# philipjesic/Distributed-Proof-Of-Work

Hardware: AMD Instinct MI355X
Metric: MD5 candidates/sec (GH/s), whole node (higher is better)
Workload: dtype u32; 1 GPU; sweep: nonce [1,2,3,4], 32 trailing zeros (unreachable), 2^36 candidates per GPU per step in the L=4 chunk segment (k >= 2^24); per-step RCCL MIN all-reduce; ntz=32, parallelism=prefix-partition x1 (workerBits=0)

## Files before the change

### distributed-proof-of-work_amd/csrc/dpow_api.cpp

```cpp
#include <hip/hip_runtime.h>
#include <stdio.h>
#include <stdlib.h>
#include <string.h>
#include <pthread.h>
#include <sched.h>
#include <sys/prctl.h>
#include <time.h>
#include <unistd.h>

#include <atomic>
#include <algorithm>
#include <chrono>
#include <mutex>
#include <string>
#include <thread>
#include <vector>

#include "../../include/dpow.h"
#include "../../include/dpow_worker.h"
#include "dpow_common.h"
#include "md5_host.h"
#include "md5_variants.h"
#include "node.h"
#include "plan.h"
#include "../../include/dpow_diag.h"


using namespace dpow;

namespace {

thread_local std::string g_last_error;

int set_error(int code, const std::string &msg) {
    g_last_error = msg;
    return code;
}

int hip_fail(hipError_t e, const char *what) {
    return set_error(DPOW_EHIP, std::string(what) + ": " + hipGetErrorString(e));
}

struct DeviceScope {
    int prev = -1;
    hipError_t e = hipSuccess;
    explicit DeviceScope(int dev) {
        if (hipGetDevice(&prev) != hipSuccess) prev = -1;
        if (prev != dev) e = hipSetDevice(dev);
        if (prev == dev) prev = -1;
    }
    ~DeviceScope() {
        if (prev >= 0) (void)hipSetDevice(prev);
    }
    DeviceScope(const DeviceScope &) = delete;
    DeviceScope &operator=(const DeviceScope &) = delete;
};

constexpr int DPOW_BOUNDED = 3;

#define DPOW_HIP(call)                                    \
    do {                                                  \
        hipError_t e_ = (call);                           \
        if (e_ != hipSuccess) return hip_fail(e_, #call); \
    } while (0)

constexpr uint64_t kBlocksPerCu = kMaxBlocksPerCu;
constexpr size_t kClaimRing = 64;
constexpr size_t kDepth = 3;
static_assert(kDepth < kClaimRing, "a claim slot is reused only after its launch completed");
constexpr size_t kRing = 8;
constexpr size_t kStaleWord = 8;
constexpr size_t kBoundWord = 16;
constexpr size_t kEarlyWord = 20;
constexpr size_t kCancelPage = 128;
static_assert(kEarlyWord * 4 + kCtrlRing * 8 <= kCancelPage, "the early-hit words fit the pinned page");
constexpr int64_t kSpinNs = 200000;
constexpr int64_t kSpinMaxNs = 4000000;
constexpr long kPollNs = 5000;
constexpr int64_t kNoDeadline = INT64_MAX;
constexpr int64_t kQueueLeadNs = 60000;
constexpr int64_t kEstFixedNs = 8000;

constexpr int kMaxDevices = 64;
std::atomic<int> g_active[kMaxDevices];
std::mutex g_ctx_mu;
std::vector<dpow_ctx *> g_ctxs;

struct ActiveSearch {
    int dev;
    explicit ActiveSearch(int d) : dev(d) { g_active[dev].fetch_add(1, std::memory_order_relaxed); }
    ~ActiveSearch() { g_active[dev].fetch_sub(1, std::memory_order_relaxed); }
};

struct LaunchSlot {
    uint64_t seq = 0;
    bool in_flight = false;
    uint64_t candidates = 0;
    uint64_t g_end = 0;
    hipStream_t stream = nullptr;
};

int64_t now_ns() {
    return std::chrono::duration_cast<std::chrono::nanoseconds>(std::chrono::steady_clock::now().time_since_epoch())
        .count();
}

struct SearchWait {
    int64_t t0 = now_ns();
    int64_t spin_ns = kSpinNs;
    long old_slack = -1;
    uint64_t node_seen = DPOW_NO_HIT;
    bool node_stop = false;
    const uint64_t *early = nullptr;
    uint64_t early_seen = DPOW_NO_HIT;
    uint64_t own_posted = DPOW_NO_HIT;
    uint64_t covered = 0;
    const uint8_t *nonce = nullptr;
    size_t nonce_len = 0;
    uint32_t ntz = 0;
    uint32_t rbits = 8, base_tb = 0;
    void lower_slack() {
        if (old_slack >= 0) return;
        const int r = prctl(PR_GET_TIMERSLACK, 0UL, 0UL, 0UL, 0UL);
        if (r <= 0) return;
        old_slack = r;
        (void)prctl(PR_SET_TIMERSLACK, 1000UL, 0UL, 0UL, 0UL);
    }
    ~SearchWait() {
        if (old_slack >= 0) (void)prctl(PR_SET_TIMERSLACK, (unsigned long)old_slack, 0UL, 0UL, 0UL);
    }
};

}

struct dpow_ctx {
    int device = 0;
    bool counted = false;
    hipStream_t stream = nullptr;
    Ctrl *d_ctrl = nullptr;
    Ctrl *d_ctrl_alloc = nullptr;
    uint32_t ctrl_idx = 0;
    unsigned long long *d_claims = nullptr;
    Snap *h_snap = nullptr;
    Snap *d_snap = nullptr;
    uint32_t *h_cancel = nullptr;
    uint32_t *d_cancel = nullptr;
    uint32_t cus = 0;
    uint64_t seq = 0;
    LaunchSlot slots[kRing];
    dpow_stats stats{};
    std::mutex bound_mu;
    bool searching = false;
    std::atomic<uint64_t> ext_bound{DPOW_NO_HIT};
    dpow_node_slot *node = nullptr;
    dpow_node_slot *d_node = nullptr;
    LaunchKnobs knobs;
    int64_t diag_t[8] = {0, 0, 0, 0, 0, 0, 0, 0};
    struct DiagLaunch {
        uint64_t seq = 0, candidates = 0, g_end = 0;
        int32_t kind = 0;
        int64_t queued = -1, seen = -1;
    };
    static constexpr size_t kDiagLaunches = 32;
    DiagLaunch diag_l[kDiagLaunches];
    size_t diag_nl = 0;
    int64_t diag_t0 = 0;
    uint64_t dev_key = 0;
    std::atomic<int64_t> last_use{0};
    bool solo = false;
};

namespace {

int retire_slot(dpow_ctx *c, LaunchSlot &s);

uint64_t *bound_word(dpow_ctx *c) { return reinterpret_cast<uint64_t *>(c->h_cancel + kBoundWord); }

int inject_bound_locked(dpow_ctx *c, uint64_t g) {
    if (g >= c->ext_bound.load(std::memory_order_relaxed)) return 0;
    c->ext_bound.store(g, std::memory_order_release);
    __atomic_store_n(bound_word(c), g, __ATOMIC_RELEASE);
    return 0;
}

int poll_node(dpow_ctx *c, SearchWait &sw) {
    dpow_node_slot *n = c->node;
    if (!n) return 0;
    const uint64_t nb = __atomic_load_n(&n->best, __ATOMIC_ACQUIRE);
    if (nb < sw.node_seen) {
        sw.node_seen = nb;
        if (nb != sw.own_posted) {
            std::lock_guard<std::mutex> g(c->bound_mu);
            uint64_t cur = c->ext_bound.load(std::memory_order_relaxed);
            if (nb < cur) c->ext_bound.store(nb, std::memory_order_release);
        }
    }
    if (!sw.node_stop && __atomic_load_n(&n->stop, __ATOMIC_ACQUIRE) != 0u) {
        sw.node_stop = true;
        __atomic_store_n(&c->h_cancel[kStaleWord], (uint32_t)c->seq, __ATOMIC_RELEASE);
    }
    return 0;
}

void poll_early(dpow_ctx *c, SearchWait &sw) {
    const uint64_t g = __atomic_load_n(sw.early, __ATOMIC_ACQUIRE);
    if (g >= sw.early_seen) return;
    sw.early_seen = g;
    if ((((uint32_t)g & 0xFFu) >> sw.rbits) != (sw.base_tb >> sw.rbits)) return;
    uint8_t sec[DPOW_MAX_SECRET];
    size_t len = 0;
    if (dpow_secret_from_index(g, sec, &len) != 0) return;
    if (!dpow_verify(sw.nonce, sw.nonce_len, sec, len, sw.ntz)) return;
    if (g < sw.own_posted) sw.own_posted = g;
    dpow_node_post(c->node, g);
    if (c->diag_t[7] < 0) c->diag_t[7] = now_ns() - sw.t0;
}

int wait_record(dpow_ctx *c, uint64_t seq, int64_t deadline, SearchWait &sw) {
    const uint32_t *p = &c->h_snap[seq % kRing].seq;
    const uint32_t want = (uint32_t)(seq + 1);
    for (uint64_t it = 1;; ++it) {
        if (__atomic_load_n(p, __ATOMIC_ACQUIRE) == want) return 1;
        const int64_t t = now_ns();
        if (t >= deadline) return 0;
        const bool spinning = t - sw.t0 < sw.spin_ns;
        if (spinning ? (it % 4096 == 0) : (it % 16 == 0)) {
            const hipError_t q = hipStreamQuery(c->slots[seq % kRing].stream);
            if (q == hipSuccess) {
                if (__atomic_load_n(p, __ATOMIC_ACQUIRE) == want) return 1;
                return set_error(DPOW_EHIP, "dpow_search: stream idle without the launch's completion record");
            }
            if (q != hipErrorNotReady) return hip_fail(q, "hipStreamQuery");
        }
        if (sw.early && (!spinning || it % 8 == 0)) poll_early(c, sw);
        if (!spinning || it % 64 == 0) {
            if (c->node) {
                const int rc = poll_node(c, sw);
                if (rc < 0) return rc;
            }
            if (c->ext_bound.load(std::memory_order_acquire) <= sw.covered) return 2;
        }
        if (spinning) {
            __builtin_ia32_pause();
        } else {
            sw.lower_slack();
            int64_t ns = kPollNs;
            if (deadline != kNoDeadline && deadline - t < ns) ns = deadline - t;
            const struct timespec ts = {0, (long)ns};
            nanosleep(&ts, nullptr);
        }
    }
}

int retire_slot(dpow_ctx *c, LaunchSlot &s) {
    if (!s.in_flight) return 0;
    const uint32_t *p = &c->h_snap[s.seq % kRing].seq;
    const uint32_t want = (uint32_t)(s.seq + 1);
    for (uint64_t it = 1; __atomic_load_n(p, __ATOMIC_ACQUIRE) != want; ++it) {
        if (it % 1024 == 0) {
            const hipError_t q = hipStreamQuery(s.stream);
            if (q == hipSuccess) {
                if (__atomic_load_n(p, __ATOMIC_ACQUIRE) == want) break;
                return set_error(DPOW_EHIP, "dpow_search: stream idle without a queued launch's completion record");
            }
            if (q != hipErrorNotReady) return hip_fail(q, "hipStreamQuery");
        }
        __builtin_ia32_pause();
    }
    s.in_flight = false;
    return 0;
}

int recent_contexts(int device) {
    const int64_t t = now_ns();
    int n = 0;
    std::lock_guard<std::mutex> g(g_ctx_mu);
    for (dpow_ctx *x : g_ctxs)
        if (x->device == device && t - x->last_use.load(std::memory_order_relaxed) < kRecentNs) ++n;
    return n;
}

int search_window(dpow_ctx *c, const uint8_t *nonce, size_t nonce_len, uint32_t ntz, uint32_t worker_byte,
                  uint32_t worker_bits, uint64_t k_begin, uint64_t k_end, uint64_t *best_global_idx,
                  uint8_t secret_out[DPOW_MAX_SECRET], size_t *secret_len) {
    WindowPlanner planner;
    int rc = planner.init(nonce, nonce_len, ntz, worker_byte, worker_bits, k_begin, k_end);
    if (rc < 0) return set_error(rc, "dpow_search: planning failed");
    const DeviceScope on_device(c->device);
    if (on_device.e != hipSuccess) return hip_fail(on_device.e, "hipSetDevice");
    if (c->device >= kMaxDevices) return set_error(DPOW_EINVAL, "dpow_search: device ordinal too large");
    const ActiveSearch active(c->device);
    SearchWait sw;
    {
        const double searches = (double)std::max(1, g_active[c->device].load(std::memory_order_relaxed));
        const double expect_ns =
            (double)expected_first_hit(ntz, remainder_bits(worker_bits)) / kEstRate * 1e9 * searches;
        sw.spin_ns = expect_ns > 2.0 * (double)kSpinMaxNs
                         ? kSpinNs
                         : (int64_t)std::min<double>(std::max<double>(2.0 * expect_ns, (double)kSpinNs),
                                                     (double)kSpinMaxNs);
    }

    {
        uint32_t *st = &c->h_cancel[kStaleWord];
        const uint32_t next = (uint32_t)(c->seq + 1);
        if ((int32_t)(next - __atomic_load_n(st, __ATOMIC_RELAXED)) > (1 << 30))
            __atomic_store_n(st, next - (1u << 30), __ATOMIC_RELAXED);
    }
    const uint64_t bound = *best_global_idx;
    const uint64_t node_best = c->node ? __atomic_load_n(&c->node->best, __ATOMIC_ACQUIRE) : DPOW_NO_HIT;
    sw.node_seen = node_best;
    const uint64_t seq0 = c->seq;
    sw.covered = k_begin << 8;
    for (int64_t &t : c->diag_t) t = -1;
    c->diag_nl = 0;
    c->diag_t0 = sw.t0;
    auto diag_queued = [c](size_t li, uint64_t seq, int32_t kind, uint64_t cands, uint64_t g_end) {
        if (li >= dpow_ctx::kDiagLaunches) return;
        c->diag_l[li] = {seq, cands, g_end, kind, now_ns(), -1};
        c->diag_nl = li + 1;
    };
    if (c->node) {
        uint64_t *ew = reinterpret_cast<uint64_t *>(c->h_cancel + kEarlyWord) + c->ctrl_idx;
        __atomic_store_n(ew, (uint64_t)DPOW_NO_HIT, __ATOMIC_RELEASE);
        sw.early = ew;
        sw.nonce = nonce;
        sw.nonce_len = nonce_len;
        sw.ntz = ntz;
        sw.rbits = remainder_bits(worker_bits);
        sw.base_tb = base_thread_byte(worker_byte, worker_bits);
    }
    size_t launched = 0, consumed = 0;
    int64_t busy_until = 0;
    PlannedLaunch pl;
    bool have = planner.next(pl);
    c->diag_t[4] = now_ns() - sw.t0;
    hipError_t e = hipSuccess;
    if (have && pl.k0) {
        LaunchSlot &k0slot = c->slots[seq0 % kRing];
        if ((rc = retire_slot(c, k0slot)) < 0) return rc;
        c->diag_t[5] = now_ns() - sw.t0;
        StartK0 k0{};
        k0.r = (uint32_t)(pl.L.i_end - pl.L.i_begin);
        k0.base_tb = pl.L.base_tb;
        k0.nblk = pl.info.nblk;
        k0.p = 4 * pl.info.w0 + pl.info.sh;
        k0.ntz = ntz;
        k0.seq = (uint32_t)(seq0 + 1);
        k0.snap = c->d_snap + seq0 % kRing;
        memcpy(k0.iv, pl.L.iv, sizeof k0.iv);
        memcpy(k0.T, pl.L.T, sizeof k0.T);
        e = search_k0(k0, c->stream);
        if (e != hipSuccess) return hip_fail(e, "search_k0");
        c->diag_t[0] = now_ns() - sw.t0;
        diag_queued(0, seq0, 0, k0.r, 1ull << 8);
        k0slot.in_flight = true;
        k0slot.seq = seq0;
        k0slot.candidates = k0.r;
        k0slot.g_end = 1ull << 8;
        k0slot.stream = c->stream;
        c->seq = seq0 + 1;
        launched = 1;
        have = planner.next(pl);
    }
    Ctrl *const ctrl = c->d_ctrl + (size_t)c->ctrl_idx * kCtrlStride;
    Ctrl *const ctrl_next = c->d_ctrl + (size_t)((c->ctrl_idx + 1) % kCtrlRing) * kCtrlStride;
    bool md5_queued = false;
    struct CtrlAdvance {
        dpow_ctx *c;
        const bool &queued;
        ~CtrlAdvance() {
            if (queued) c->ctrl_idx = (c->ctrl_idx + 1) % kCtrlRing;
        }
    } ctrl_advance{c, md5_queued};
    const uint64_t bound0 = node_best < bound ? node_best : bound;
    struct BoundWindow {
        dpow_ctx *c;
        BoundWindow(dpow_ctx *cc, uint64_t start) : c(cc) {
            std::lock_guard<std::mutex> g(c->bound_mu);
            c->ext_bound.store(start, std::memory_order_relaxed);
            __atomic_store_n(bound_word(c), (uint64_t)DPOW_NO_HIT, __ATOMIC_RELEASE);
            c->searching = true;
        }
        ~BoundWindow() {
            std::lock_guard<std::mutex> g(c->bound_mu);
            c->searching = false;
        }
    } bound_window(c, node_best);

    uint32_t done_target = 0;
    struct StaleOnReturn {
        dpow_ctx *c;
        const size_t &launched, &consumed;
        ~StaleOnReturn() {
            if (consumed < launched) __atomic_store_n(&c->h_cancel[kStaleWord], (uint32_t)c->seq, __ATOMIC_RELEASE);
        }
    } stale_on_return{c, launched, consumed};
    uint64_t best = bound;
    int status = DPOW_EXHAUSTED;
    auto consume = [&](size_t lj) -> int {
        const uint64_t seq = seq0 + lj;
        const int rc = wait_record(c, seq, kNoDeadline, sw);
        if (rc < 0) return rc;
        if (rc == 2) return DPOW_BOUNDED;
        LaunchSlot &slot = c->slots[seq % kRing];
        const Snap &sn = c->h_snap[seq % kRing];
        slot.in_flight = false;
        c->stats.launches++;
        c->stats.candidates += slot.candidates;
        if (sn.t_start != 0ull && sn.t_end >= sn.t_start)
            c->stats.kernel_ms += (double)(sn.t_end - sn.t_start) * kRealtimeNs * 1e-6;
        if (consumed == 0) c->diag_t[2] = now_ns() - sw.t0;
        if (lj < dpow_ctx::kDiagLaunches) c->diag_l[lj].seen = now_ns();
        consumed = lj + 1;
        if (c->node) {
            const int prc = poll_node(c, sw);
            if (prc < 0) return prc;
        }
        if (sn.best < bound) {
            const uint64_t eb = c->ext_bound.load(std::memory_order_acquire);
            if (sn.best >= eb) return eb <= slot.g_end ? DPOW_BOUNDED : DPOW_EXHAUSTED;
            best = sn.best;
            return DPOW_FOUND;
        }
        if (sn.stop != 0u || sw.node_stop || __atomic_load_n(c->h_cancel, __ATOMIC_ACQUIRE) != 0u)
            return DPOW_CANCELLED;
        sw.covered = slot.g_end;
        if (c->ext_bound.load(std::memory_order_acquire) <= sw.covered) return DPOW_BOUNDED;
        return DPOW_EXHAUSTED;
    };
    while (status == DPOW_EXHAUSTED && have) {
        if (sw.node_stop) {
            status = DPOW_CANCELLED;
            break;
        }
        const size_t li = launched;
        if (li - consumed >= kDepth) {
            const int r = consume(consumed);
            if (r < 0) return r;
            if (r != DPOW_EXHAUSTED) status = r;
            continue;
        }
        if (li > consumed && busy_until - now_ns() > kQueueLeadNs) {
            const size_t lj = consumed;
            const int w = wait_record(c, seq0 + lj, busy_until - kQueueLeadNs, sw);
            if (w < 0) return w;
            if (w == 2) {
                status = DPOW_BOUNDED;
                continue;
            }
            if (w == 1) {
                const int r = consume(lj);
                if (r < 0) return r;
                if (r != DPOW_EXHAUSTED) status = r;
                continue;
            }
        }
        {
            const uint64_t eb = c->ext_bound.load(std::memory_order_acquire);
            if ((pl.info.k_begin << 8) >= (eb < bound ? eb : bound)) break;
        }
        const uint64_t seq = seq0 + li;
        LaunchSlot &slot = c->slots[seq % kRing];
        if ((rc = retire_slot(c, slot)) < 0) return rc;
        if (!md5_queued) c->diag_t[6] = now_ns() - sw.t0;
        Launch &L = pl.L;
        uint64_t active = (uint64_t)std::max(1, g_active[c->device].load(std::memory_order_relaxed));
        if (active == 1 && !c->solo && now_ns() - sw.t0 < kYoungNs) {
            const int recent = recent_contexts(c->device);
            if (recent > 1) active = (uint64_t)recent;
        }
        const uint64_t share = grid_share(active, c->knobs);
        cap_shared_launch(planner, pl, active, c->knobs);
        uint64_t worker_blocks = 0;
        rc = size_search_launch(pl, ntz, c->cus, share, c->knobs, &worker_blocks, active);
        if (rc < 0) return set_error(rc, "dpow_search: launch grid leaves a claim counter without waves");
        done_target += (uint32_t)worker_blocks;
        L.claim = c->d_claims + (li % kClaimRing) * kClaimSlot;
        L.done_target = done_target;
        L.ctrl = ctrl;
        L.ctrl_next = ctrl_next;
        L.bound0 = bound0;
        L.cancel = c->d_cancel;
        L.stale = c->d_cancel + kStaleWord;
        L.ext_bound = reinterpret_cast<const unsigned long long *>(c->d_cancel + kBoundWord);
        L.snap = c->d_snap + seq % kRing;
        L.seq = (uint32_t)(seq + 1);
        L.node_best = c->d_node ? reinterpret_cast<const unsigned long long *>(&c->d_node->best) : nullptr;
        L.node_stop = c->d_node ? &c->d_node->stop : nullptr;
        L.early = c->d_node ? reinterpret_cast<unsigned long long *>(c->d_cancel + kEarlyWord) + c->ctrl_idx : nullptr;
        e = search_launch((int)pl.info.nblk, (int)pl.info.w0, (int)pl.info.sh, L, (uint32_t)(worker_blocks + 1),
                          c->stream);
        if (e != hipSuccess) return hip_fail(e, "search_launch");
        if (!md5_queued) c->diag_t[1] = now_ns() - sw.t0;
        diag_queued(li, seq, 1, L.i_end - L.i_begin, pl.info.k_end << 8);
        md5_queued = true;
        slot.seq = seq;
        slot.in_flight = true;
        slot.candidates = L.i_end - L.i_begin;
        slot.g_end = pl.info.k_end << 8;
        slot.stream = c->stream;
        c->seq = seq + 1;
        ++launched;
        const int64_t t = now_ns();
        busy_until = std::max(busy_until, t) + kEstFixedNs +
                     (int64_t)((double)slot.candidates * (double)active / kEstRate * 1e9);
        have = planner.next(pl);
    }
    while (status == DPOW_EXHAUSTED && consumed < launched) {
        const int r = consume(consumed);
        if (r < 0) return r;
        status = r;
    }
    if (status == DPOW_BOUNDED) status = DPOW_EXHAUSTED;
    c->diag_t[3] = now_ns() - sw.t0;

    if (status == DPOW_FOUND) {
        dpow_secret_from_index(best, secret_out, secret_len);
        if (!dpow_verify(nonce, nonce_len, secret_out, *secret_len, ntz)) {
            *secret_len = 0;
            return set_error(DPOW_EVERIFY, "dpow_search: kernel hit failed host MD5 verification");
        }
        *best_global_idx = best;
    }
    return status;
}

struct PageEntry {
    void *page;
    bool foreign;
    std::vector<dpow_ctx *> holders;
    char *dev[kMaxDevices] = {};
};
std::mutex g_page_mu;
std::vector<PageEntry> g_pages;

void page_drop_locked(size_t i) {
    if (!g_pages[i].foreign) (void)hipHostUnregister(g_pages[i].page);
    g_pages.erase(g_pages.begin() + (long)i);
}

hipError_t page_hold_locked(dpow_ctx *c, void *page, char **dev) {
    PageEntry *pe = nullptr;
    for (PageEntry &x : g_pages)
        if (x.page == page) {
            pe = &x;
            break;
        }
    if (!pe) {
        hipError_t e = hipHostRegister(page, 4096, hipHostRegisterMapped | hipHostRegisterPortable);
        bool foreign = false;
        if (e == hipErrorHostMemoryAlreadyRegistered) {
            (void)hipGetLastError();
            e = hipSuccess;
            foreign = true;
        }
        if (e != hipSuccess) return e;
        g_pages.push_back(PageEntry{page, foreign, {}, {}});
        pe = &g_pages.back();
    }
    if (!pe->dev[c->device]) {
        void *d = nullptr;
        const hipError_t e = hipHostGetDevicePointer(&d, page, 0);
        if (e != hipSuccess) {
            if (pe->holders.empty()) page_drop_locked((size_t)(pe - g_pages.data()));
            return e;
        }
        pe->dev[c->device] = static_cast<char *>(d);
    }
    if (std::find(pe->holders.begin(), pe->holders.end(), c) == pe->holders.end()) pe->holders.push_back(c);
    *dev = pe->dev[c->device];
    return hipSuccess;
}

void pages_release_ctx(dpow_ctx *c) {
    std::lock_guard<std::mutex> g(g_page_mu);
    for (size_t i = g_pages.size(); i-- > 0;) {
        auto &h = g_pages[i].holders;
        h.erase(std::remove(h.begin(), h.end(), c), h.end());
        if (h.empty()) page_drop_locked(i);
    }
}

hipError_t prepare_device(int device) {
    static std::mutex mu;
    static bool prepared[kMaxDevices] = {};
    std::lock_guard<std::mutex> g(mu);
    if (device < kMaxDevices && prepared[device]) return hipSuccess;
    const hipError_t e = search_prepare();
    if (e == hipSuccess && device < kMaxDevices) prepared[device] = true;
    return e;
}

}

extern "C" {

const char *dpow_last_error(void) { return g_last_error.c_str(); }
int dpow_abi_version(void) { return DPOW_ABI_VERSION; }

int dpow_device_count(void) {
    int n = 0;
    if (hipGetDeviceCount(&n) != hipSuccess) {
        (void)hipGetLastError();
        return 0;
    }
    return n;
}

int dpow_open(int device, dpow_ctx **out) {
    if (!out) return set_error(DPOW_EINVAL, "dpow_open: out is NULL");
    *out = nullptr;
    int n = 0;
    hipError_t e = hipGetDeviceCount(&n);
    if (e != hipSuccess || n == 0) return set_error(DPOW_EHIP, "dpow_open: no HIP device visible");
    if (device < 0 || device >= n) return set_error(DPOW_EINVAL, "dpow_open: bad device ordinal");
    const DeviceScope on_device(device);
    if (on_device.e != hipSuccess) return hip_fail(on_device.e, "hipSetDevice");
    dpow_ctx *c = new (std::nothrow) dpow_ctx();
    if (!c) return set_error(DPOW_ENOMEM, "dpow_open: out of memory");
    c->device = device;
    hipDeviceProp_t prop;
    if ((e = hipGetDeviceProperties(&prop, device)) != hipSuccess) {
        delete c;
        return hip_fail(e, "hipGetDeviceProperties");
    }
    c->cus = (uint32_t)prop.multiProcessorCount;
    {
        char bus[64] = {0};
        if (hipDeviceGetPCIBusId(bus, (int)sizeof bus - 1, device) != hipSuccess) {
            (void)hipGetLastError();
            snprintf(bus, sizeof bus, "ordinal-%d-pid-%d", device, (int)getpid());
        }
        uint64_t h = 1469598103934665603ull;
        for (const char *q = bus; *q; ++q) h = (h ^ (uint8_t)*q) * 1099511628211ull;
        c->dev_key = h | 1ull;
    }
    if (const char *pw = getenv("DPOW_DIAG_POLL_WB")) c->knobs.poll_wb = (uint32_t)std::max(0, atoi(pw));
    if (const char *pw = getenv("DPOW_DIAG_BPC")) c->knobs.bpc = (uint32_t)std::max(0, atoi(pw));
    if (const char *pw = getenv("DPOW_DIAG_CPW")) c->knobs.cpw = (uint32_t)std::max(0, atoi(pw));
    if (const char *pw = getenv("DPOW_DIAG_SHARE_LAUNCH_US")) c->knobs.share_launch_us = (uint32_t)std::max(0, atoi(pw));
    if (const char *pw = getenv("DPOW_DIAG_SHARE_MAX")) c->knobs.share_max = (uint32_t)std::max(0, atoi(pw));
    if (const char *pw = getenv("DPOW_DIAG_MIN_CHUNK")) {
        const uint32_t v = (uint32_t)std::max(0, atoi(pw));
        if (v && !(v & (v - 1))) c->knobs.min_chunk = v;
    }
    if ((e = hipStreamCreateWithFlags(&c->stream, hipStreamNonBlocking)) != hipSuccess ||
        (e = hipMalloc(&c->d_ctrl_alloc, 2 * kCtrlRing * kCtrlStride * sizeof(Ctrl))) != hipSuccess ||
        (e = hipMalloc(&c->d_claims, kClaimRing * kClaimSlot * sizeof(unsigned long long))) != hipSuccess ||
        (e = hipHostMalloc(&c->h_snap, kRing * sizeof(Snap), hipHostMallocCoherent | hipHostMallocMapped)) !=
            hipSuccess ||
        (e = hipHostGetDevicePointer(reinterpret_cast<void **>(&c->d_snap), c->h_snap, 0)) != hipSuccess ||
        (e = hipHostMalloc(&c->h_cancel, kCancelPage, hipHostMallocCoherent | hipHostMallocMapped)) != hipSuccess ||
        (e = hipHostGetDevicePointer(reinterpret_cast<void **>(&c->d_cancel), c->h_cancel, 0)) != hipSuccess) {
        dpow_close(c);
        return hip_fail(e, "dpow_open: allocation");
    }
    {
        const uintptr_t rb = kCtrlRing * kCtrlStride * sizeof(Ctrl);
        c->d_ctrl = reinterpret_cast<Ctrl *>((reinterpret_cast<uintptr_t>(c->d_ctrl_alloc) + rb - 1) & ~(rb - 1));
    }
    memset(c->h_snap, 0, kRing * sizeof(Snap));
    memset(c->h_cancel, 0, kCancelPage);
    *bound_word(c) = DPOW_NO_HIT;
    if ((e = context_init(c->d_ctrl, kCtrlRing * kCtrlStride, c->d_claims, (uint32_t)(kClaimRing * kClaimSlot),
                          c->stream)) != hipSuccess ||
        (e = hipStreamSynchronize(c->stream)) != hipSuccess) {
        dpow_close(c);
        return hip_fail(e, "dpow_open: control state");
    }
    if ((e = prepare_device(device)) != hipSuccess) {
        dpow_close(c);
        return hip_fail(e, "dpow_open: loading the search kernels");
    }
    c->last_use.store(now_ns(), std::memory_order_relaxed);
    {
        std::lock_guard<std::mutex> g(g_ctx_mu);
        g_ctxs.push_back(c);
        c->counted = true;
    }
    *out = c;
    return 0;
}

void dpow_close(dpow_ctx *c) {
    if (!c) return;
    if (c->counted) {
        std::lock_guard<std::mutex> g(g_ctx_mu);
        g_ctxs.erase(std::remove(g_ctxs.begin(), g_ctxs.end(), c), g_ctxs.end());
    }
    const DeviceScope on_device(c->device);
    if (c->stream) (void)hipStreamSynchronize(c->stream);
    c->node = c->d_node = nullptr;
    pages_release_ctx(c);
    if (c->d_ctrl_alloc) (void)hipFree(c->d_ctrl_alloc);
    if (c->d_claims) (void)hipFree(c->d_claims);
    if (c->h_snap) (void)hipHostFree(c->h_snap);
    if (c->h_cancel) (void)hipHostFree(c->h_cancel);
    if (c->stream) (void)hipStreamDestroy(c->stream);
    delete c;
}

volatile uint32_t *dpow_cancel_flag(dpow_ctx *c) { return c ? c->h_cancel : nullptr; }
void *dpow_stream(dpow_ctx *c) { return c ? (void *)c->stream : nullptr; }
int dpow_device(dpow_ctx *c) { return c ? c->device : -1; }

int dpow_geometry(dpow_ctx *c, uint32_t *cus, uint32_t *blocks_per_cu, uint32_t *threads_per_block) {
    if (!c) return set_error(DPOW_EINVAL, "dpow_geometry: ctx is NULL");
    if (cus) *cus = c->cus;
    if (blocks_per_cu) *blocks_per_cu = (uint32_t)kBlocksPerCu;
    if (threads_per_block) *threads_per_block = kBlockThreads;
    return 0;
}

int dpow_get_stats(dpow_ctx *c, dpow_stats *out) {
    if (!c || !out) return set_error(DPOW_EINVAL, "dpow_get_stats: NULL argument");
    *out = c->stats;
    return 0;
}

void dpow_reset_stats(dpow_ctx *c) {
    if (!c) return;
    c->stats = dpow_stats{};
}

int dpow_search_bound(dpow_ctx *c, uint64_t global_idx) {
    if (!c) return set_error(DPOW_EINVAL, "dpow_search_bound: ctx is NULL");
    std::lock_guard<std::mutex> g(c->bound_mu);
    if (!c->searching) return 0;
    return inject_bound_locked(c, global_idx);
}

int dpow_node_attach(dpow_ctx *c, dpow_node_slot *slot) {
    if (!c) return set_error(DPOW_EINVAL, "dpow_node_attach: ctx is NULL");
    if (!slot) {
        c->node = c->d_node = nullptr;
        return 0;
    }
    if (((uintptr_t)slot & 7u) != 0u) return set_error(DPOW_EINVAL, "dpow_node_attach: slot not 8-byte aligned");
    if (c->device >= kMaxDevices) return set_error(DPOW_EINVAL, "dpow_node_attach: device ordinal too large");
    const DeviceScope on_device(c->device);
    if (on_device.e != hipSuccess) return hip_fail(on_device.e, "hipSetDevice");
    const uintptr_t pg = 4096;
    const bool one_page = (((uintptr_t)slot & (pg - 1)) + sizeof(dpow_node_slot)) <= pg;
    char *dev = nullptr;
    {
        std::lock_guard<std::mutex> g(g_page_mu);
        for (uintptr_t a = (uintptr_t)slot & ~(pg - 1); a < (uintptr_t)slot + sizeof(dpow_node_slot); a += pg) {
            char *d = nullptr;
            const hipError_t e = page_hold_locked(c, (void *)a, &d);
            if (e != hipSuccess) return hip_fail(e, "dpow_node_attach: hipHostRegister");
            if (!dev) dev = d;
        }
    }
    void *d = dev + ((uintptr_t)slot & (pg - 1));
    if (!one_page) DPOW_HIP(hipHostGetDevicePointer(&d, slot, 0));
    c->node = slot;
    c->d_node = (dpow_node_slot *)d;
    return 0;
}

int dpow_node_release(void *mem, size_t len) {
    if (!mem || !len) return 0;
    const uintptr_t pg = 4096;
    const uintptr_t lo = (uintptr_t)mem & ~(pg - 1), hi = (uintptr_t)mem + len;
    std::lock_guard<std::mutex> g(g_page_mu);
    for (const PageEntry &pe : g_pages) {
        const uintptr_t p = (uintptr_t)pe.page;
        if (p < lo || p >= hi) continue;
        for (dpow_ctx *h : pe.holders)
            if (h->node && (uintptr_t)h->node < p + pg && (uintptr_t)h->node + sizeof(dpow_node_slot) > p)
                return set_error(DPOW_EINVAL, "dpow_node_release: a context is still attached to a slot in the range");
    }
    for (size_t i = g_pages.size(); i-- > 0;) {
        const uintptr_t p = (uintptr_t)g_pages[i].page;
        if (p < lo || p >= hi) continue;
        for (dpow_ctx *h : g_pages[i].holders) {
            const DeviceScope on_device(h->device);
            const hipError_t e = hipStreamSynchronize(h->stream);
            if (e != hipSuccess) return hip_fail(e, "dpow_node_release: hipStreamSynchronize");
        }
        page_drop_locked(i);
    }
    return 0;
}

void dpow_node_slot_reset(dpow_node_slot *slot) {
    if (!slot) return;
    __atomic_store_n(&slot->stop, 0u, __ATOMIC_RELAXED);
    __atomic_store_n(&slot->best, DPOW_NO_HIT, __ATOMIC_RELEASE);
}

void dpow_node_post(dpow_node_slot *slot, uint64_t global_idx) {
    if (!slot) return;
    uint64_t cur = __atomic_load_n(&slot->best, __ATOMIC_RELAXED);
    while (global_idx < cur &&
           !__atomic_compare_exchange_n(&slot->best, &cur, global_idx, true, __ATOMIC_ACQ_REL, __ATOMIC_RELAXED)) {
    }
}

int dpow_node_vote(dpow_node_vote_entry *votes, uint32_t rank, uint32_t world, uint64_t epoch, const int64_t in[3],
                   int64_t out[3], int64_t timeout_ns) {
    return dpow::node_vote(votes, rank, world, epoch, in, out, timeout_ns, nullptr);
}

}

int dpow::node_vote(dpow_node_vote_entry *votes, uint32_t rank, uint32_t world, uint64_t epoch, const int64_t in[3],
                    int64_t out[3], int64_t timeout_ns, const uint32_t *abort_flag) {
    if (!votes || !in || !out || world == 0 || rank >= world || epoch == 0)
        return set_error(DPOW_EINVAL, "dpow_node_vote: bad argument");
    dpow_node_vote_entry &mine = votes[2 * rank + (epoch & 1)];
    for (int i = 0; i < 3; ++i) __atomic_store_n(&mine.v[i], in[i], __ATOMIC_RELAXED);
    __atomic_store_n(&mine.epoch, epoch, __ATOMIC_RELEASE);
    int64_t acc[3] = {in[0], in[1], in[2]};
    const int64_t t0 = now_ns();
    constexpr int64_t kVoteSpinNs = 500000;
    long old_slack = -1;
    struct SlackRestore {
        long &old;
        ~SlackRestore() {
            if (old >= 0) (void)prctl(PR_SET_TIMERSLACK, (unsigned long)old, 0UL, 0UL, 0UL);
        }
    } slack_restore{old_slack};
    for (uint32_t r = 0; r < world; ++r) {
        if (r == rank) continue;
        const dpow_node_vote_entry &e = votes[2 * r + (epoch & 1)];
        for (uint64_t it = 0; __atomic_load_n(&e.epoch, __ATOMIC_ACQUIRE) != epoch; ++it) {
            if (abort_flag && it % 64 == 0 && __atomic_load_n(abort_flag, __ATOMIC_ACQUIRE) != 0u) return DPOW_CANCELLED;
            if (it % 64 != 0 || now_ns() - t0 < std::min(kVoteSpinNs, timeout_ns)) {
                __builtin_ia32_pause();
                continue;
            }
            if (now_ns() - t0 > timeout_ns)
                return set_error(DPOW_EPROTO, "dpow_node_vote: rank " + std::to_string(r) + " did not vote at epoch " +
                                                  std::to_string(epoch));
            if (old_slack < 0) {
                const int sl = prctl(PR_GET_TIMERSLACK, 0UL, 0UL, 0UL, 0UL);
                if (sl > 0) {
                    old_slack = sl;
                    (void)prctl(PR_SET_TIMERSLACK, 1000UL, 0UL, 0UL, 0UL);
                }
            }
            const struct timespec d = {0, 2000};
            nanosleep(&d, nullptr);
        }
        for (int i = 0; i < 3; ++i) {
            const int64_t v = __atomic_load_n(&e.v[i], __ATOMIC_RELAXED);
            if (v < acc[i]) acc[i] = v;
        }
    }
    for (int i = 0; i < 3; ++i) out[i] = acc[i];
    return 0;
}

extern "C" int dpow_node_mine(dpow_ctx *c, dpow_node_slot *slot, dpow_node_vote_entry *votes, uint32_t rank,
                              uint32_t world, uint64_t *epoch, int64_t vote_timeout_ns, const uint8_t *nonce,
                              size_t nonce_len, uint32_t ntz, uint64_t k_begin, uint64_t k_limit, uint64_t first_k,
                              uint64_t batch_k, uint64_t *best_global_idx, uint8_t secret_out[DPOW_MAX_SECRET],
                              size_t *secret_len, uint32_t *batches) {
    return dpow::node_mine(c, slot, votes, rank, world, epoch, vote_timeout_ns, nonce, nonce_len, ntz, k_begin, k_limit,
                           first_k, batch_k, best_global_idx, secret_out, secret_len, batches, false, 0);
}

int dpow::node_mine(dpow_ctx *c, dpow_node_slot *slot, dpow_node_vote_entry *votes, uint32_t rank, uint32_t world,
                    uint64_t *epoch, int64_t vote_timeout_ns, const uint8_t *nonce, size_t nonce_len, uint32_t ntz,
                    uint64_t k_begin, uint64_t k_limit, uint64_t first_k, uint64_t batch_k, uint64_t *best_global_idx,
                    uint8_t secret_out[DPOW_MAX_SECRET], size_t *secret_len, uint32_t *batches, bool abandon_on_cancel,
                    int role) {
    if (!c || !slot || !epoch || !best_global_idx || !secret_out || !secret_len || !batches)
        return set_error(DPOW_EINVAL, "dpow_node_mine: NULL argument");
    if (world == 0 || (world & (world - 1)) != 0 || world > 256 || rank >= world)
        return set_error(DPOW_EINVAL, "dpow_node_mine: world must be a power of two <= 256, rank < world");
    if (batch_k == 0 || k_limit > DPOW_K_LIMIT) return set_error(DPOW_EINVAL, "dpow_node_mine: bad window");
    const uint32_t wbits = (uint32_t)__builtin_ctz(world);
    *batches = 0;
    *secret_len = 0;
    int err = dpow_node_attach(c, slot);
    if (err < 0) dpow_node_stop(slot);
    uint64_t k = k_begin, window = first_k ? first_k : batch_k;
    uint8_t sec[DPOW_MAX_SECRET];
    size_t slen = 0;
    uint64_t own = DPOW_NO_HIT;
    int status = DPOW_EXHAUSTED;
    while (k < k_limit) {
        const uint64_t ke = k_limit - k > window ? k + window : k_limit;
        window = batch_k;
        int rc = DPOW_EXHAUSTED;
        if (err == 0) {
            uint64_t best = DPOW_NO_HIT;
            if (role == 2) rc = DPOW_EXHAUSTED;
            else rc = dpow_search(c, nonce, nonce_len, ntz, role == 1 ? 0 : rank, role == 1 ? 0 : wbits, k, ke, &best,
                                  sec, &slen);
            if (rc < 0) {
                err = rc;
                dpow_node_stop(slot);
            } else if (rc == DPOW_FOUND && best < own) {
                own = best;
                memcpy(secret_out, sec, slen);
                *secret_len = slen;
            }
        }
        const int64_t running =
            (err != 0 || rc == DPOW_CANCELLED || __atomic_load_n(c->h_cancel, __ATOMIC_ACQUIRE) != 0u) ? 0 : 1;
        const uint64_t posted = __atomic_load_n(&slot->best, __ATOMIC_ACQUIRE);
        const int64_t in[3] = {(int64_t)(own < posted ? own : posted), running, err != 0 ? 0 : 1};
        int64_t out[3] = {in[0], in[1], in[2]};
        if (abandon_on_cancel && err == 0 && __atomic_load_n(c->h_cancel, __ATOMIC_ACQUIRE) != 0u) {
            dpow_node_stop(slot);
            status = DPOW_CANCELLED;
            break;
        }
        if (votes) {
            const int vr = node_vote(votes, rank, world, ++*epoch, in, out, vote_timeout_ns,
                                     abandon_on_cancel ? c->h_cancel : nullptr);
            if (vr == DPOW_CANCELLED) {
                dpow_node_stop(slot);
                status = DPOW_CANCELLED;
                break;
            }
            if (vr < 0) {
                err = err ? err : vr;
                out[2] = 0;
            }
        }
        ++*batches;
        if (out[2] == 0) {
            status = err ? err : set_error(DPOW_EPROTO, "dpow_node_mine: another rank's search failed");
            break;
        }
        if ((uint64_t)out[0] != DPOW_NO_HIT) {
            *best_global_idx = (uint64_t)out[0];
            if ((uint64_t)out[0] != own) dpow_secret_from_index((uint64_t)out[0], secret_out, secret_len);
            status = DPOW_FOUND;
            break;
        }
        if (out[1] == 0) {
            status = DPOW_CANCELLED;
            break;
        }
        k = ke;
    }
    if (c->node == slot) c->node = c->d_node = nullptr;
    if (status != DPOW_FOUND) *secret_len = 0;
    return status;
}

int dpow::fail(int code, const char *msg) { return set_error(code, msg); }

uint64_t dpow::device_key(const dpow_ctx *c) { return c ? c->dev_key : 0; }

void dpow::set_solo(dpow_ctx *c, bool solo) {
    if (c) c->solo = solo;
}

extern "C" {

int dpow_diag_node_post_at(dpow_node_slot *slot, uint64_t global_idx, int64_t t_ns) {
    if (!slot) return set_error(DPOW_EINVAL, "dpow_diag_node_post_at: slot is NULL");
    struct Poster {
        std::mutex mu;
        std::vector<std::pair<int64_t, std::pair<dpow_node_slot *, uint64_t>>> q;
        std::atomic<int> pending{0};
        bool alive = false;
    };
    static Poster *const P = new Poster;
    std::lock_guard<std::mutex> g(P->mu);
    P->q.push_back({t_ns, {slot, global_idx}});
    P->pending.fetch_add(1, std::memory_order_release);
    if (!P->alive) {
        P->alive = true;
        std::thread([]() {
            auto mono = []() {
                struct timespec ts;
                clock_gettime(CLOCK_MONOTONIC, &ts);
                return (int64_t)ts.tv_sec * 1000000000 + ts.tv_nsec;
            };
            int64_t idle_since = mono();
            for (;;) {
                if (P->pending.load(std::memory_order_acquire) == 0) {
                    if (mono() - idle_since > 2000000000) {
                        std::lock_guard<std::mutex> g2(P->mu);
                        if (P->pending.load(std::memory_order_acquire) == 0) {
                            P->alive = false;
                            return;
                        }
                    }
                    __builtin_ia32_pause();
                    continue;
                }
                std::pair<int64_t, std::pair<dpow_node_slot *, uint64_t>> w;
                int rest = 0;
                {
                    std::lock_guard<std::mutex> g2(P->mu);
                    auto it = std::min_element(P->q.begin(), P->q.end(),
                                               [](const auto &x, const auto &y) { return x.first < y.first; });
                    w = *it;
                    P->q.erase(it);
                    rest = P->pending.fetch_sub(1, std::memory_order_acq_rel) - 1;
                }
                bool requeued = false;
                for (;;) {
                    const int64_t left = w.first - mono();
                    if (left <= 0) break;
                    if (P->pending.load(std::memory_order_acquire) > rest) {
                        std::lock_guard<std::mutex> g2(P->mu);
                        P->q.push_back(w);
                        P->pending.fetch_add(1, std::memory_order_release);
                        requeued = true;
                        break;
                    }
                    if (left > 100000) {
                        const struct timespec d = {0, (long)std::min<int64_t>(left - 50000, 50000)};
                        nanosleep(&d, nullptr);
                    } else {
                        __builtin_ia32_pause();
                    }
                }
                if (requeued) continue;
                dpow_node_post(w.second.first, w.second.second);
                idle_since = mono();
            }
        }).detach();
    }
    return 0;
}

int dpow_diag_vote_latency(uint32_t world, int reps, double *last_us, double *all_us) {
    if (world < 2 || world > 256 || reps < 1 || !last_us || !all_us)
        return set_error(DPOW_EINVAL, "dpow_diag_vote_latency: world in [2, 256], reps >= 1, outputs non-NULL");
    void *mem = aligned_alloc(64, (size_t)2 * world * sizeof(dpow_node_vote_entry));
    if (!mem) return set_error(DPOW_EINVAL, "dpow_diag_vote_latency: out of memory");
    memset(mem, 0, (size_t)2 * world * sizeof(dpow_node_vote_entry));
    auto *votes = static_cast<dpow_node_vote_entry *>(mem);
    cpu_set_t allowed;
    CPU_ZERO(&allowed);
    std::vector<int> cpus;
    if (sched_getaffinity(0, sizeof allowed, &allowed) == 0)
        for (int i = 0; i < CPU_SETSIZE; ++i) {
            if (!CPU_ISSET(i, &allowed)) continue;
            char path[96];
            snprintf(path, sizeof path, "/sys/devices/system/cpu/cpu%d/topology/thread_siblings_list", i);
            if (FILE *f = fopen(path, "r")) {
                int first = -1;
                const int n = fscanf(f, "%d", &first);
                fclose(f);
                if (n == 1 && first != i) continue;
            }
            cpus.push_back(i);
        }
    auto pin = [&](uint32_t r) {
        if (cpus.empty()) return;
        cpu_set_t one;
        CPU_ZERO(&one);
        CPU_SET(cpus[(size_t)r * cpus.size() / world], &one);
        (void)pthread_setaffinity_np(pthread_self(), sizeof one, &one);
    };
    std::atomic<int> go{0};
    std::vector<std::atomic<int64_t>> done_at(world);
    for (auto &d : done_at) d.store(0);
    std::atomic<int> failed{0};
    std::vector<std::thread> others;
    for (uint32_t r = 1; r < world; ++r)
        others.emplace_back([&, r]() {
            pin(r);
            for (int rep = 1; rep <= reps; ++rep) {
                while (go.load(std::memory_order_acquire) < rep) __builtin_ia32_pause();
                if (failed.load()) break;
                const int64_t in[3] = {(int64_t)(1000 + r), 1, 1};
                int64_t out[3];
                if (dpow_node_vote(votes, r, world, (uint64_t)rep, in, out, 1000000000) != 0) failed.store(1);
                done_at[r].store(now_ns(), std::memory_order_release);
                while (go.load(std::memory_order_acquire) == rep) __builtin_ia32_pause();
            }
        });
    cpu_set_t caller;
    const bool have_caller = pthread_getaffinity_np(pthread_self(), sizeof caller, &caller) == 0;
    pin(0);
    std::vector<double> last, all;
    int64_t t_prev_done = 0;
    for (int rep = 1; rep <= reps && !failed.load(); ++rep) {
        go.store(rep, std::memory_order_release);
        for (uint32_t r = 1; r < world; ++r)
            while (__atomic_load_n(&votes[2 * r + (rep & 1)].epoch, __ATOMIC_ACQUIRE) != (uint64_t)rep &&
                   !failed.load())
                __builtin_ia32_pause();
        for (const int64_t t_wait = now_ns(); now_ns() - t_wait < 2000;) __builtin_ia32_pause();
        const int64_t t0 = now_ns();
        const int64_t in[3] = {1000, 1, 1};
        int64_t out[3];
        if (dpow_node_vote(votes, 0, world, (uint64_t)rep, in, out, 1000000000) != 0 || out[0] != 1000) failed.store(1);
        const int64_t t1 = now_ns();
        int64_t t_all = t1;
        for (uint32_t r = 1; r < world && !failed.load(); ++r) {
            int64_t t;
            while ((t = done_at[r].load(std::memory_order_acquire)) <= t_prev_done && !failed.load())
                __builtin_ia32_pause();
            t_all = std::max(t_all, t);
        }
        t_prev_done = t_all;
        last.push_back((t1 - t0) / 1e3);
        all.push_back((t_all - t0) / 1e3);
    }
    go.store(reps + 1, std::memory_order_release);
    for (auto &t : others) t.join();
    if (have_caller) (void)pthread_setaffinity_np(pthread_self(), sizeof caller, &caller);
    free(mem);
    if (failed.load() || last.empty()) return set_error(DPOW_EPROTO, "dpow_diag_vote_latency: a vote failed");
    std::sort(last.begin(), last.end());
    std::sort(all.begin(), all.end());
    *last_us = last[last.size() / 2];
    *all_us = all[all.size() / 2];
    return 0;
}

void dpow_node_stop(dpow_node_slot *slot) {
    if (slot) __atomic_store_n(&slot->stop, 1u, __ATOMIC_RELEASE);
}

int dpow_secret_from_index(uint64_t g, uint8_t secret_out[DPOW_MAX_SECRET], size_t *secret_len) {
    if (!secret_out || !secret_len) return set_error(DPOW_EINVAL, "dpow_secret_from_index: NULL argument");
    if (g == DPOW_NO_HIT) return set_error(DPOW_EINVAL, "dpow_secret_from_index: no hit");
    size_t n = 0;
    secret_out[n++] = (uint8_t)(g & 0xFF);
    for (uint64_t k = g >> 8; k; k >>= 8) secret_out[n++] = (uint8_t)(k & 0xFF);
    *secret_len = n;
    return 0;
}

void dpow_md5(const uint8_t *msg, size_t len, uint8_t digest_out[16]) { md5_digest(msg, len, digest_out); }

uint32_t dpow_trailing_zero_nibbles(const uint8_t digest[16]) { return digest_trailing_zero_nibbles(digest); }

int dpow_verify(const uint8_t *nonce, size_t nonce_len, const uint8_t *secret, size_t secret_len, uint32_t ntz) {
    std::vector<uint8_t> msg(nonce_len + secret_len);
    if (nonce_len) memcpy(msg.data(), nonce, nonce_len);
    if (secret_len) memcpy(msg.data() + nonce_len, secret, secret_len);
    uint8_t d[16];
    md5_digest(msg.data(), msg.size(), d);
    return digest_trailing_zero_nibbles(d) >= ntz ? 1 : 0;
}

int dpow_plan_window(const uint8_t *nonce, size_t nonce_len, uint32_t ntz, uint32_t worker_byte,
                     uint32_t worker_bits, uint64_t k_begin, uint64_t k_end, dpow_plan_launch *out,
                     size_t max_launches) {
    std::vector<PlannedLaunch> plan;
    int n = plan_window(nonce, nonce_len, ntz, worker_byte, worker_bits, k_begin, k_end, plan);
    if (n < 0) return set_error(n, "dpow_plan_window: bad arguments");
    for (size_t i = 0; i < plan.size() && i < max_launches && out; ++i) out[i] = plan[i].info;
    return n;
}

int dpow_plan_candidate(const uint8_t *nonce, size_t nonce_len, uint32_t worker_byte, uint32_t worker_bits,
                        uint64_t local_idx, uint32_t iv_out[4], uint32_t words_out[32], uint32_t *nblk_out) {
    if (!iv_out || !words_out || !nblk_out) return set_error(DPOW_EINVAL, "dpow_plan_candidate: NULL argument");
    const uint64_t k = local_idx >> remainder_bits(worker_bits);
    const uint32_t clen = chunk_len_of(k);
    uint64_t k_first = clen == 0 ? k : 1ull << (8 * (clen - 1));
    if (const uint64_t w2 = word2_period((uint32_t)(nonce_len % 64) % 4))
        if (k_first < k / w2 * w2) k_first = k / w2 * w2;
    std::vector<PlannedLaunch> plan;
    int n = plan_window(nonce, nonce_len, 0, worker_byte, worker_bits, k_first, k + 1, plan);
    if (n != 1) return set_error(n < 0 ? n : DPOW_EINVAL, "dpow_plan_candidate: bad arguments");
    for (int w = 0; w < 4; ++w) iv_out[w] = plan[0].L.iv[w];
    memset(words_out, 0, 32 * sizeof(uint32_t));
    candidate_words(plan[0], local_idx, words_out);
    *nblk_out = plan[0].info.nblk;
    return 0;
}

int dpow_diag_launch_geometry(const uint8_t *nonce, size_t nonce_len, uint32_t ntz, uint32_t worker_byte,
                              uint32_t worker_bits, uint64_t k_begin, uint64_t k_end, uint32_t cus, uint32_t share,
                              dpow_diag_launch *out, size_t max_launches) {
    if (cus == 0 || share == 0) return set_error(DPOW_EINVAL, "dpow_diag_launch_geometry: cus and share must be > 0");
    WindowPlanner planner;
    const int rc = planner.init(nonce, nonce_len, ntz, worker_byte, worker_bits, k_begin, k_end);
    if (rc < 0) return set_error(rc, "dpow_diag_launch_geometry: bad arguments");
    PlannedLaunch pl;
    size_t n = 0;
    const LaunchKnobs policy{};
    while (planner.next(pl)) {
        if (pl.k0) continue;
        cap_shared_launch(planner, pl, share, policy);
        uint64_t wblocks = 0;
        const int r = size_search_launch(pl, ntz, cus, grid_share(share, policy), policy, &wblocks, share);
        if (r < 0) return set_error(r, "dpow_diag_launch_geometry: launch grid leaves a claim counter without waves");
        if (out && n < max_launches) {
            dpow_diag_launch &d = out[n];
            d.k_begin = pl.info.k_begin;
            d.k_end = pl.info.k_end;
            d.i_begin = pl.L.i_begin;
            d.i_end = pl.L.i_end;
            d.wb_begin = pl.L.wb_begin;
            d.n_wblocks = pl.L.n_wblocks;
            d.n_big = pl.L.n_big;
            d.n_chunks = pl.L.n_chunks;
            d.worker_blocks = wblocks;
            d.chunk = pl.L.chunk;
            d.chunk_tail = pl.L.chunk_tail;
            d.rbits = pl.L.rbits;
            d.wave_block = kWaveBlock;
            d.n_static = pl.L.n_static;
            d.poll_wb = pl.L.poll_wb;
        }
        ++n;
    }
    return (int)n;
}

int dpow_diag_node_alias(dpow_ctx *c, void **cached, void **lookup) {
    if (!c || !cached || !lookup) return set_error(DPOW_EINVAL, "dpow_diag_node_alias: NULL argument");
    if (!c->node) return set_error(DPOW_EINVAL, "dpow_diag_node_alias: no slot attached");
    const DeviceScope on_device(c->device);
    if (on_device.e != hipSuccess) return hip_fail(on_device.e, "hipSetDevice");
    *cached = c->d_node;
    DPOW_HIP(hipHostGetDevicePointer(lookup, c->node, 0));
    return 0;
}

int dpow_diag_search_times(dpow_ctx *c, int64_t out[8]) {
    if (!c || !out) return set_error(DPOW_EINVAL, "dpow_diag_search_times: NULL argument");
    for (int i = 0; i < 8; ++i) out[i] = c->diag_t[i];
    return 0;
}

int dpow_diag_search_launches(dpow_ctx *c, int64_t *t0_ns, dpow_diag_launch_time *out, size_t max_launches) {
    if (!c || !t0_ns) return set_error(DPOW_EINVAL, "dpow_diag_search_launches: NULL argument");
    *t0_ns = c->diag_t0;
    const size_t n = c->diag_nl;
    for (size_t i = 0; out && i < n && i < max_launches; ++i) {
        const dpow_ctx::DiagLaunch &d = c->diag_l[i];
        dpow_diag_launch_time &o = out[i];
        o.seq = d.seq;
        o.kind = d.kind;
        o.queued_ns = d.queued;
        o.seen_ns = d.seen;
        o.candidates = d.candidates;
        o.g_end = d.g_end;
        const Snap &sn = c->h_snap[d.seq % kRing];
        const bool rec = __atomic_load_n(&sn.seq, __ATOMIC_ACQUIRE) == (uint32_t)(d.seq + 1);
        o.recorded = rec ? 1 : 0;
        o.t_start_tick = rec ? sn.t_start : 0;
        o.t_end_tick = rec ? sn.t_end : 0;
        o.best = rec ? sn.best : DPOW_NO_HIT;
    }
    return (int)n;
}

int dpow_diag_clock_sync(dpow_ctx *c, int reps, int64_t *offset_ns) {
    if (!c || !offset_ns || reps < 1) return set_error(DPOW_EINVAL, "dpow_diag_clock_sync: bad argument");
    const DeviceScope on_device(c->device);
    if (on_device.e != hipSuccess) return hip_fail(on_device.e, "hipSetDevice");
    hipError_t e = hipStreamSynchronize(c->stream);
    if (e != hipSuccess) return hip_fail(e, "dpow_diag_clock_sync: hipStreamSynchronize");
    unsigned long long *h = nullptr, *d = nullptr;
    if ((e = hipHostMalloc(&h, 64, hipHostMallocCoherent | hipHostMallocMapped)) != hipSuccess)
        return hip_fail(e, "dpow_diag_clock_sync: hipHostMalloc");
    if ((e = hipHostGetDevicePointer(reinterpret_cast<void **>(&d), h, 0)) != hipSuccess) {
        (void)hipHostFree(h);
        return hip_fail(e, "dpow_diag_clock_sync: hipHostGetDevicePointer");
    }
    int64_t best = INT64_MAX;
    int rc = 0;
    for (int r = 0; r < reps && rc == 0; ++r) {
        __atomic_store_n(h, 0ull, __ATOMIC_RELEASE);
        if ((e = clock_probe(d, c->stream)) != hipSuccess) {
            rc = hip_fail(e, "dpow_diag_clock_sync: clock_probe");
            break;
        }
        const int64_t t_launch = now_ns();
        unsigned long long tick = 0;
        int64_t t = 0;
        while ((tick = __atomic_load_n(h, __ATOMIC_ACQUIRE)) == 0ull) {
            t = now_ns();
            if (t - t_launch > 1000000000) {
                rc = set_error(DPOW_EHIP, "dpow_diag_clock_sync: the probe's stamp never arrived");
                break;
            }
            __builtin_ia32_pause();
        }
        if (rc) break;
        t = now_ns();
        const int64_t off = t - (int64_t)((double)tick * kRealtimeNs);
        if (off < best) best = off;
    }
    e = hipStreamSynchronize(c->stream);
    if (rc == 0 && e != hipSuccess) rc = hip_fail(e, "dpow_diag_clock_sync: hipStreamSynchronize");
    (void)hipHostFree(h);
    if (rc == 0) *offset_ns = best;
    return rc;
}

uint64_t dpow_diag_blocks_per_cu(uint64_t candidates, uint32_t ntz, uint32_t worker_bits) {
    return launch_blocks_per_cu(candidates, ntz, remainder_bits(worker_bits));
}

int dpow_diag_dword_test(const uint8_t *nonce, size_t nonce_len, uint32_t ntz, uint64_t k, uint32_t iv_d,
                         uint32_t state_d) {
    std::vector<PlannedLaunch> plan;
    const int n = plan_window(nonce, nonce_len, ntz, 0, 0, k, k + 1, plan);
    if (n != 1) return set_error(n < 0 ? n : DPOW_EINVAL, "dpow_diag_dword_test: bad arguments");
    const Launch &L = plan[0].L;
    const uint32_t nblk = plan[0].info.nblk;
    if (nblk == 1 && iv_d != L.iv[3]) return set_error(DPOW_EINVAL, "dpow_diag_dword_test: iv_d != iv[3]");
    const uint32_t D = iv_d + state_d;
    const bool pre = use_d_equality(nblk, ntz) ? state_d == L.deq : D <= L.dle;
    return pre && (D & L.dmask) == 0u ? 1 : 0;
}

int dpow_search(dpow_ctx *c, const uint8_t *nonce, size_t nonce_len, uint32_t ntz, uint32_t worker_byte,
                uint32_t worker_bits, uint64_t k_begin, uint64_t k_end, uint64_t *best_global_idx,
                uint8_t secret_out[DPOW_MAX_SECRET], size_t *secret_len) {
    if (!c || !best_global_idx || !secret_out || !secret_len)
        return set_error(DPOW_EINVAL, "dpow_search: NULL argument");
    if (nonce_len && !nonce) return set_error(DPOW_EINVAL, "dpow_search: nonce is NULL");
    if (worker_byte > 255u) return set_error(DPOW_EINVAL, "dpow_search: worker_byte > 255");
    if (k_end > DPOW_K_LIMIT) return set_error(DPOW_ERANGE, "dpow_search: k_end beyond DPOW_K_LIMIT");
    *secret_len = 0;
    c->stats.searches++;
    c->last_use.store(now_ns(), std::memory_order_relaxed);
    if (k_begin >= k_end) return DPOW_EXHAUSTED;
    dpow_node_slot *const node = c->node;
    if (node && __atomic_load_n(&node->stop, __ATOMIC_ACQUIRE) != 0u) return DPOW_CANCELLED;
    if (__atomic_load_n(c->h_cancel, __ATOMIC_ACQUIRE) != 0u) {
        dpow_node_stop(node);
        return DPOW_CANCELLED;
    }
    const int status = search_window(c, nonce, nonce_len, ntz, worker_byte, worker_bits, k_begin, k_end,
                                     best_global_idx, secret_out, secret_len);
    if (node) {
        if (status == DPOW_FOUND) dpow_node_post(node, *best_global_idx);
        else if (status != DPOW_EXHAUSTED) dpow_node_stop(node);
    }
    return status;
}

}
```

### distributed-proof-of-work_amd/csrc/dpow_common.h

```cpp
#pragma once

#include <stdint.h>

#if defined(__HIPCC__)
#include <hip/hip_runtime.h>
#define DPOW_HD __host__ __device__ __forceinline__
#else
#define DPOW_HD inline
#endif

namespace dpow {

constexpr uint32_t kMd5K[64] = {
    0xd76aa478, 0xe8c7b756, 0x242070db, 0xc1bdceee, 0xf57c0faf, 0x4787c62a, 0xa8304613, 0xfd469501,
    0x698098d8, 0x8b44f7af, 0xffff5bb1, 0x895cd7be, 0x6b901122, 0xfd987193, 0xa679438e, 0x49b40821,
    0xf61e2562, 0xc040b340, 0x265e5a51, 0xe9b6c7aa, 0xd62f105d, 0x02441453, 0xd8a1e681, 0xe7d3fbc8,
    0x21e1cde6, 0xc33707d6, 0xf4d50d87, 0x455a14ed, 0xa9e3e905, 0xfcefa3f8, 0x676f02d9, 0x8d2a4c8a,
    0xfffa3942, 0x8771f681, 0x6d9d6122, 0xfde5380c, 0xa4beea44, 0x4bdecfa9, 0xf6bb4b60, 0xbebfbc70,
    0x289b7ec6, 0xeaa127fa, 0xd4ef3085, 0x04881d05, 0xd9d4d039, 0xe6db99e5, 0x1fa27cf8, 0xc4ac5665,
    0xf4292244, 0x432aff97, 0xab9423a7, 0xfc93a039, 0x655b59c3, 0x8f0ccc92, 0xffeff47d, 0x85845dd1,
    0x6fa87e4f, 0xfe2ce6e0, 0xa3014314, 0x4e0811a1, 0xf7537e82, 0xbd3af235, 0x2ad7d2bb, 0xeb86d391};

constexpr uint32_t kMd5IV[4] = {0x67452301u, 0xefcdab89u, 0x98badcfeu, 0x10325476u};

constexpr int md5_shift(int i) {
    return (i < 16)   ? (i % 4 == 0 ? 7 : i % 4 == 1 ? 12 : i % 4 == 2 ? 17 : 22)
           : (i < 32) ? (i % 4 == 0 ? 5 : i % 4 == 1 ? 9 : i % 4 == 2 ? 14 : 20)
           : (i < 48) ? (i % 4 == 0 ? 4 : i % 4 == 1 ? 11 : i % 4 == 2 ? 16 : 23)
                      : (i % 4 == 0 ? 6 : i % 4 == 1 ? 10 : i % 4 == 2 ? 15 : 21);
}

constexpr int md5_word(int i) {
    return (i < 16) ? i : (i < 32) ? (1 + 5 * i) % 16 : (i < 48) ? (5 + 3 * i) % 16 : (7 * i) % 16;
}

constexpr uint32_t kBop3F = 0xCA;
constexpr uint32_t kBop3G = 0xE4;
constexpr uint32_t kBop3H = 0x96;
constexpr uint32_t kBop3I = 0x39;



#ifndef DPOW_NC
#define DPOW_NC 2
#endif
constexpr int kNC = DPOW_NC;
constexpr int kWaveBlock = 64 * kNC;
constexpr int kBlockThreads = 256;
constexpr uint32_t kClaimCounters = 8;
constexpr uint32_t kClaimStride = 16;
constexpr uint32_t kClaimSlot = kClaimCounters * kClaimStride;

constexpr unsigned long long kNoHit = 0x7FFFFFFFFFFFFFFFull;
struct Ctrl {
    unsigned long long best;
    uint32_t stop;
    uint32_t pad0_;
    unsigned long long pad1_[14];
    uint32_t done;
    uint32_t pad2_[31];
};
constexpr uint32_t kCtrlLine = 256;
constexpr uint32_t kCtrlRing = 4;
constexpr uint32_t kCtrlStride = kCtrlLine / sizeof(Ctrl);
static_assert((kCtrlRing & (kCtrlRing - 1)) == 0 && kCtrlLine % sizeof(Ctrl) == 0, "the ring is aligned to its size");
static_assert(sizeof(Ctrl) == 256 && __builtin_offsetof(Ctrl, done) == 128, "done on its own line");

struct Snap {
    unsigned long long best;
    uint32_t stop;
    uint32_t seq;
    unsigned long long t_start, t_end;
};
constexpr double kRealtimeNs = 10.0;

struct Launch {
    uint32_t iv[4];
    uint32_t T[32];
    uint32_t KT[128];
    uint64_t i_begin;
    uint64_t i_end;
    uint64_t wb_begin;
    uint64_t n_wblocks;
    uint32_t rbits;
    uint32_t base_tb;
    uint32_t dmask;
    uint32_t dle;
    uint32_t deq;
    uint32_t ntz;
    uint32_t seg_first;
    uint32_t done_target;
    uint32_t chunk;
    uint32_t chunk_tail;
    uint64_t n_big;
    uint64_t n_chunks;
    uint64_t n_head;
    uint64_t n_static;
    uint32_t poll_wb;
    uint32_t reserved0;
    unsigned long long *claim;
    Ctrl *ctrl;
    Ctrl *ctrl_next;
    const uint32_t *cancel;
    const uint32_t *stale;
    const unsigned long long *ext_bound;
    Snap *snap;
    uint32_t seq;
    uint32_t pad1;
    unsigned long long bound0;
    const unsigned long long *node_best;
    const uint32_t *node_stop;
    unsigned long long *early;
    uint32_t lspan;
    uint32_t seg0;
};

DPOW_HD uint32_t chunk_len_lt24(uint32_t k) { return (k != 0u) + (k > 0xFFu) + (k > 0xFFFFu); }

DPOW_HD void lseg_deltas(uint32_t l, uint32_t &d0, uint32_t &d1, uint32_t &dlen) {
    const uint64_t pad = 0x80ull << (8 * (1 + l));
    d0 = (uint32_t)pad - 0x8000u;
    d1 = (uint32_t)(pad >> 32);
    dlen = 8u * l;
}

constexpr uint32_t kLsegBase = 0xFFFFFFF0u;
DPOW_HD uint32_t seg_id(uint64_t k) {
    return k >> 24 ? (uint32_t)(k >> 24) : kLsegBase + chunk_len_lt24((uint32_t)k);
}

DPOW_HD uint32_t tail_nibble_mask(uint32_t n) {
    const uint32_t pos[8] = {24, 28, 16, 20, 8, 12, 0, 4};
    uint32_t m = 0;
    for (uint32_t j = 0; j < n && j < 8; ++j) m |= 0xFu << pos[j];
    return m;
}

DPOW_HD uint32_t tail_prefilter_le(uint32_t n) {
    const uint32_t e = (n < 8 ? n : 8) & ~1u;
    return e == 0 ? 0xFFFFFFFFu : e >= 8 ? 0u : (0xFFFFFFFFu >> (4 * e));
}

DPOW_HD bool use_d_equality(uint32_t nblk, uint32_t ntz) { return nblk == 1 && ntz >= 8; }

DPOW_HD uint32_t bswap32(uint32_t x) {
    return (x >> 24) | ((x >> 8) & 0xFF00u) | ((x << 8) & 0xFF0000u) | (x << 24);
}

DPOW_HD uint32_t trailing_zero_nibbles(uint32_t A, uint32_t B, uint32_t C, uint32_t D) {
    const uint32_t w[4] = {bswap32(D), bswap32(C), bswap32(B), bswap32(A)};
    uint32_t n = 0;
    for (int j = 0; j < 4; ++j) {
        if (w[j] == 0) { n += 8; continue; }
        uint32_t x = w[j];
        while ((x & 0xF) == 0) { x >>= 4; ++n; }
        break;
    }
    return n;
}

DPOW_HD uint32_t lane_offset(uint32_t rbits, uint32_t lane) {
    return rbits >= 6 ? lane : ((lane & ((1u << rbits) - 1u)) | ((lane >> rbits) << 8));
}
DPOW_HD uint32_t wave_uniform_v(uint64_t i0, uint32_t rbits, uint32_t base_tb) {
    const uint64_t R = 1ull << rbits;
    return base_tb | (uint32_t)(i0 & (R - 1)) | ((uint32_t)((i0 >> rbits) & 0xFFFFFFu) << 8);
}
DPOW_HD void seg_word_deltas(uint32_t t1, uint32_t t2, uint32_t seg, uint32_t seg_first, uint32_t sh,
                             uint32_t &d1, uint32_t &d2) {
    const uint64_t t = ((uint64_t)t2 << 32) | t1;
    const uint64_t x = t + ((uint64_t)(seg - seg_first) << (8 * sh));
    d1 = (uint32_t)x - t1;
    d2 = (uint32_t)(x >> 32) - t2;
}

DPOW_HD uint64_t global_of_local(uint64_t i, uint32_t rbits, uint32_t base_tb) {
    const uint64_t R = 1ull << rbits;
    return ((i >> rbits) << 8) | (uint64_t)(base_tb | (uint32_t)(i & (R - 1)));
}

}
```

### distributed-proof-of-work_amd/csrc/md5_dispatch.cpp

```cpp
#include "md5_variants.h"

namespace dpow {

hipError_t search_launch(int nblk, int w0, int sh, const Launch &L, uint32_t grid, hipStream_t stream) {
    if (!variant_exists(nblk, w0, sh)) return hipErrorInvalidValue;
    if (L.seg0 == kLsegBase) {
        if (sh != 0) return hipErrorInvalidValue;
        return nblk == 1 ? variant_launch_1_0_ls(w0, L, grid, stream)
                         : variant_launch_2_0_ls(w0, L, grid, stream);
    }
#define DPOW_CASE(n, s) \
    if (nblk == n && sh == s) return variant_launch_##n##_##s(w0, L, grid, stream);
    DPOW_CASE(1, 0) DPOW_CASE(1, 1) DPOW_CASE(1, 2) DPOW_CASE(1, 3)
    DPOW_CASE(2, 0) DPOW_CASE(2, 1) DPOW_CASE(2, 2) DPOW_CASE(2, 3)
#undef DPOW_CASE
    return hipErrorInvalidValue;
}

hipError_t search_occupancy(int nblk, int w0, int sh, int *blocks_per_cu) {
    if (!variant_exists(nblk, w0, sh)) return hipErrorInvalidValue;
#define DPOW_CASE(n, s) \
    if (nblk == n && sh == s) return variant_occupancy_##n##_##s(w0, blocks_per_cu);
    DPOW_CASE(1, 0) DPOW_CASE(1, 1) DPOW_CASE(1, 2) DPOW_CASE(1, 3)
    DPOW_CASE(2, 0) DPOW_CASE(2, 1) DPOW_CASE(2, 2) DPOW_CASE(2, 3)
#undef DPOW_CASE
    return hipErrorInvalidValue;
}

hipError_t search_prepare() {
    hipError_t e = search_k0_prepare();
#define DPOW_PREP(n, s) \
    if (e == hipSuccess) e = variant_prepare_##n##_##s();
    DPOW_PREP(1, 0) DPOW_PREP(1, 1) DPOW_PREP(1, 2) DPOW_PREP(1, 3)
    DPOW_PREP(2, 0) DPOW_PREP(2, 1) DPOW_PREP(2, 2) DPOW_PREP(2, 3)
    DPOW_PREP(1, 0_ls) DPOW_PREP(2, 0_ls)
#undef DPOW_PREP
    return e;
}

}
```

### distributed-proof-of-work_amd/csrc/md5_search_kernel.h

```cpp
#pragma once
#include <hip/hip_runtime.h>

#include "dpow_common.h"

#ifndef DPOW_VLS
#define DPOW_VLS 0
#endif
#if DPOW_VLS
#define DPOW_KNS lsk
#else
#define DPOW_KNS k
#endif

namespace dpow {
namespace DPOW_KNS {

#define DPOW_DEV __device__ __forceinline__
#define DPOW_DEV_CONST __host__ __device__ constexpr

#ifndef DPOW_NUM_SGPR
#define DPOW_NUM_SGPR 72
#endif
#ifndef DPOW_NUM_SGPR_LONG
#define DPOW_NUM_SGPR_LONG 96
#endif
#ifndef DPOW_NUM_SGPR_W15
#define DPOW_NUM_SGPR_W15 100
#endif
constexpr int kSgprLongW0 = 8;
constexpr int kWatchSleep = 16;
#ifndef DPOW_POLL_WB
#define DPOW_POLL_WB 16
#endif
constexpr bool kXcdRetire = DPOW_VLS != 0;
constexpr bool kStaticFirst = DPOW_VLS != 0;
#ifndef DPOW_WAVE_TRACE
#define DPOW_WAVE_TRACE 0
#endif
#if DPOW_WAVE_TRACE
constexpr uint32_t kTraceWaves = 8192;
constexpr uint32_t kTraceFields = 8;
static __device__ unsigned long long g_wave_trace[kTraceWaves * kTraceFields];
#endif

template <int I>
DPOW_DEV uint32_t md5_fn(uint32_t x, uint32_t y, uint32_t z) {
    constexpr int r = I / 16;
    constexpr uint32_t tt = r == 0 ? kBop3F : r == 1 ? kBop3G : r == 2 ? kBop3H : kBop3I;
    return __builtin_amdgcn_bitop3_b32(x, y, z, tt);
}


struct KConst {
    uint32_t v[128];
};

static_assert(DPOW_POLL_WB > 0, "the chunk loop polls per group of wave-blocks");
template <int NBLK, int W0, int SH>
DPOW_DEV_CONST bool seg_word(int m) {
    return (SH == 0 && m == W0 + 1) || (SH == 3 && m == W0 + 2 && m != 16 * NBLK - 2) ||
           (DPOW_VLS && SH == 0 && (m == W0 + 1 || m == 16 * NBLK - 2));
}

struct NarrowKnobs {
    bool on;
    int lead, cap, poll, sgpr;
};
constexpr NarrowKnobs narrow_knobs(int nblk, int w0) {
    if (nblk == 1) {
        switch (w0) {
            case 1: case 2: case 3: case 5: case 6: case 11:
                    return {true, 2, 0, 0, 1};
            case 4: return {true, 1, 0, -1, -1};
            case 7: return {true, 2, 0, -1, 1};
            case 8: return {true, 3, 0, 0, -1};
            case 9: return {true, 4, 0, -1, -1};
            case 10: return {true, 2, 0, 0, -1};
            default: return {false, 0, 0, -1, -1};
        }
    }
    switch (w0) {
        case 12: return {true, 3, 0, 0, -1};
        case 13: return {true, 3, 0, -1, -1};
        case 14: return {true, 2, 24, -1, -1};
        case 15: return {true, 2, 0, 0, -1};
        default: return {false, 0, 0, -1, -1};
    }
}
#ifndef DPOW_NLEAD
#define DPOW_NLEAD 0
#endif
#ifndef DPOW_NCAP
#define DPOW_NCAP 0
#endif
#ifndef DPOW_NPOLL
#define DPOW_NPOLL -1
#endif
#ifndef DPOW_NSGPR
#define DPOW_NSGPR 0
#endif

constexpr int pipe_lead(int nblk, int w0, int sh, bool narrow = false) {
    if (narrow) {
        const int lead = DPOW_NLEAD > 0 ? DPOW_NLEAD : narrow_knobs(nblk, w0).lead;
        if (lead > 0) return lead;
    }
    if (nblk == 1) {
        switch (w0 * 4 + sh) {
            case 0 * 4 + 0: return 2;
            case 0 * 4 + 3: return 2;
            case 2 * 4 + 0: return 3;
            case 2 * 4 + 1: return 1;
            case 2 * 4 + 2: return 1;
            case 3 * 4 + 0: return 3;
            case 3 * 4 + 1: return 3;
            case 3 * 4 + 2: return 3;
            case 3 * 4 + 3: return 1;
            case 4 * 4 + 0: return 2;
            case 4 * 4 + 3: return 2;
            case 6 * 4 + 3: return 2;
            case 8 * 4 + 3: return 3;
            case 9 * 4 + 0: return 2;
            case 9 * 4 + 1: return 3;
            case 9 * 4 + 2: return 3;
            case 9 * 4 + 3: return 3;
            case 10 * 4 + 3: return 5;
            default: return 4;
        }
    }
    switch (w0 * 4 + sh) {
        case 12 * 4 + 3: return 1;
        case 14 * 4 + 1: return 2;
        case 14 * 4 + 2: return 2;
        case 14 * 4 + 3: return 1;
        case 15 * 4 + 0: return 2;
        case 15 * 4 + 1: return 2;
        case 15 * 4 + 2: return 2;
        case 15 * 4 + 3: return 1;
        default: return 4;
    }
}

template <int NBLK, int W0, int SH, bool KS = true>
struct VgprK {
    static constexpr bool kNarrow = SH == 3 && !KS;
    static constexpr int kEnd0 = NBLK == 1 ? 62 : 64;
    static constexpr int kLead = pipe_lead(NBLK, W0, SH, kNarrow);
    static constexpr int kI0 = W0 + kLead < kEnd0 ? W0 + kLead : kEnd0;
    static constexpr bool run(int blk, int i) { return !(blk == NBLK - 1 && i >= 62); }
    static constexpr bool seg(int blk, int i) { return seg_word<NBLK, W0, SH>(16 * blk + md5_word(i)) && run(blk, i); }
    static constexpr bool eligible(int blk, int i) {
        const int m = 16 * blk + md5_word(i);
        const bool zero = m > W0 + 2 && m != 16 * NBLK - 2;
        const bool lane = m == W0 || (SH != 0 && m == W0 + 1);
        const bool piped = blk > 0 || i >= kI0;
        return !zero && !lane && piped && run(blk, i) && !seg(blk, i);
    }
    static constexpr int rank(int blk, int i) {
        int r = 0;
        for (int b = 0; b < NBLK; ++b)
            for (int j = 0; j < 64; ++j) {
                if (b == blk && j == i) return r;
                if (eligible(b, j)) ++r;
            }
        return r;
    }
    static constexpr int count() { return rank(NBLK, 0); }
    static constexpr int count_seg() {
        int r = 0;
        for (int b = 0; b < NBLK; ++b)
            for (int j = 0; j < 64; ++j) r += seg(b, j) ? 1 : 0;
        return r;
    }
    static constexpr bool kCap24 = NBLK == 1 && ((W0 == 7 && (SH == 1 || SH == 2)) || (SH == 3 && (W0 == 4 || W0 == 5)));
    static constexpr int kNarrowCap = DPOW_NCAP > 0 ? DPOW_NCAP : narrow_knobs(NBLK, W0).cap;
    static constexpr int kCap = kNarrow && kNarrowCap > 0 ? kNarrowCap
                                : kCap24 ? 24
                                : NBLK == 1 ? (SH == 0 ? 24 : SH == 3 ? 14 : 18)
                                            : (SH == 3 ? 20 : 26);
    static constexpr bool use(int blk, int i) {
        return seg(blk, i) || (eligible(blk, i) && rank(blk, i) < kCap - count_seg());
    }
};

template <int NBLK, int W0, int SH, int BLK, int I, bool KS>
DPOW_DEV void kconst_init(KConst &kc, const Launch &L) {
    if constexpr (BLK < NBLK) {
        if constexpr (VgprK<NBLK, W0, SH, KS>::use(BLK, I))
            asm("v_mov_b32 %0, %1" : "=v"(kc.v[64 * BLK + I]) : "s"(L.KT[64 * BLK + I]));
        if constexpr (I + 1 < 64) kconst_init<NBLK, W0, SH, BLK, I + 1, KS>(kc, L);
        else kconst_init<NBLK, W0, SH, BLK + 1, 0, KS>(kc, L);
    }
}

template <int W0, int SH>
DPOW_DEV void seg_deltas(const Launch &L, uint32_t seg, uint32_t &d1, uint32_t &d2) {
    seg_word_deltas(L.T[W0 + 1], L.T[W0 + 2], seg, L.seg_first, SH, d1, d2);
}

template <int NBLK, int W0>
DPOW_DEV uint32_t seg_add(int m, const uint32_t (&d)[3]) {
    return m == 16 * NBLK - 2 ? d[2] : m == W0 + 1 ? d[0] : d[1];
}

template <int NBLK, int W0, int SH>
DPOW_DEV void seg_all_deltas(const Launch &L, uint32_t sg, uint32_t &d0, uint32_t (&d)[3]) {
    d0 = d[0] = d[1] = d[2] = 0u;
    if (sg >= kLsegBase) {
        if constexpr (SH == 0 && DPOW_VLS) {
            lseg_deltas((sg - kLsegBase) & 3u, d0, d[0], d[2]);
            if constexpr (W0 + 1 == 16 * NBLK - 2) {
                d[2] += d[0];
                d[0] = 0u;
            }
        }
    } else {
        seg_deltas<W0, SH>(L, sg, d[0], d[1]);
    }
}

template <int NBLK, int W0, int SH, int BLK, int I, bool KS>
DPOW_DEV void kconst_seg(KConst &kc, const Launch &L, const uint32_t (&d)[3]) {
    if constexpr (BLK < NBLK) {
        if constexpr (VgprK<NBLK, W0, SH, KS>::seg(BLK, I)) {
            constexpr int m = 16 * BLK + md5_word(I);
            const uint32_t k = L.KT[64 * BLK + I] + seg_add<NBLK, W0>(m, d);
            asm volatile("v_mov_b32 %0, %1" : "=v"(kc.v[64 * BLK + I]) : "s"(k));
        }
        if constexpr (I + 1 < 64) kconst_seg<NBLK, W0, SH, BLK, I + 1, KS>(kc, L, d);
        else kconst_seg<NBLK, W0, SH, BLK + 1, 0, KS>(kc, L, d);
    }
}

template <bool KSPAN>
struct VarWords {
    static constexpr bool kSpan = KSPAN;
    uint32_t lo_s[kNC];
    uint32_t lo_v;
    uint32_t hi_s[kNC];
    uint32_t lane_k;
    const KConst *kc;
    uint32_t seg_d[3];
};

template <int NBLK, int W0, int SH, int BLK, int I, bool KS>
struct StepWord {
    static constexpr int m = 16 * BLK + md5_word(I);
    static constexpr bool zero_word = m > W0 + 2 && m != 16 * NBLK - 2;
    static constexpr bool per_lane = m == W0 || (SH == 3 && KS && m == W0 + 1);
    static constexpr bool vgpr_k = VgprK<NBLK, W0, SH, KS>::use(BLK, I);
    static constexpr bool seg = seg_word<NBLK, W0, SH>(m);
    static DPOW_DEV uint32_t km(const Launch &L, const VarWords<KS> &v, int j) {
        uint32_t k = zero_word ? kMd5K[I] : vgpr_k ? v.kc->v[64 * BLK + I] : L.KT[64 * BLK + I];
        if constexpr (seg && !vgpr_k) k += seg_add<NBLK, W0>(m, v.seg_d);
        if constexpr (m == W0) k = (k + v.lo_s[j]) + v.lo_v;
        if constexpr (SH != 0 && m == W0 + 1) {
            k += v.hi_s[j];
            if constexpr (SH == 3 && KS) k += v.lane_k;
        }
        return k;
    }
};

template <int NBLK, int W0, int SH, int BLK, int I, int IE, int NCAND, class V>
DPOW_DEV void md5_steps(uint32_t (&x)[4][kNC], const Launch &L, const V &v) {
    if constexpr (I < IE) {
        constexpr int ai = (64 - I) % 4, bi = (ai + 1) % 4, ci = (ai + 2) % 4, di = (ai + 3) % 4;
        constexpr int s = md5_shift(I);
#pragma unroll
        for (int j = 0; j < NCAND; ++j) {
            const uint32_t km = StepWord<NBLK, W0, SH, BLK, I, V::kSpan>::km(L, v, j);
            const uint32_t f = md5_fn<I>(x[bi][j], x[ci][j], x[di][j]);
            x[ai][j] = x[bi][j] + __builtin_rotateleft32(x[ai][j] + f + km, s);
        }
        md5_steps<NBLK, W0, SH, BLK, I + 1, IE, NCAND>(x, L, v);
    }
}

namespace pipe {

template <int I>
constexpr uint32_t tt() {
    return I / 16 == 0 ? kBop3F : I / 16 == 1 ? kBop3G : I / 16 == 2 ? kBop3H : kBop3I;
}

template <int I> struct Roles {
    static constexpr int a = (64 - I) % 4, b = (a + 1) % 4, c = (a + 2) % 4, d = (a + 3) % 4;
};

#define DPOW_PAD_R "s_nop 0\n\t"
#define DPOW_PAD_A "s_nop 2\n\t"

#define DPOW_PIPE_BODY                                        \
    "v_bitop3_b32 %[fp], %[pb], %[pc], %[pd] bitop3:%[tt]\n\t" \
    "v_alignbit_b32 %[rq], %[tq], %[tq], %[sq]\n\t" DPOW_PAD_R \
    "v_add3_u32 %[tp], %[pa], %[fp], %[kp]\n\t" DPOW_PAD_A     \
    "v_add_u32_e32 %[qb], %[qc], %[rq]\n\t"                   \
    "v_alignbit_b32 %[tp], %[tp], %[tp], %[sp]\n\t" DPOW_PAD_R \
    "v_bitop3_b32 %[fq], %[qb], %[qc], %[qd] bitop3:%[tt]\n\t" \
    "v_add_u32_e32 %[pa], %[pb], %[tp]\n\t"                   \
    "v_add3_u32 %[tq], %[qa], %[fq], %[kq]\n\t" DPOW_PAD_A

#define DPOW_PIPE_PRO                                         \
    "v_bitop3_b32 %[fp], %[pb], %[pc], %[pd] bitop3:%[tt]\n\t" \
    "v_add3_u32 %[tp], %[pa], %[fp], %[kp]\n\t" DPOW_PAD_A     \
    "v_bitop3_b32 %[fq], %[qb], %[qc], %[qd] bitop3:%[tt]\n\t" \
    "v_alignbit_b32 %[tp], %[tp], %[tp], %[sp]\n\t" DPOW_PAD_R \
    "v_add_u32_e32 %[pa], %[pb], %[tp]\n\t"                   \
    "v_add3_u32 %[tq], %[qa], %[fq], %[kq]\n\t" DPOW_PAD_A

template <int NBLK, int W0, int SH, int BLK, int I, int J, class V>
DPOW_DEV void body(uint32_t (&x)[4][kNC], uint32_t &tq, const Launch &L, const V &v) {
    using R = Roles<I>;
    using W = StepWord<NBLK, W0, SH, BLK, I, V::kSpan>;
    const uint32_t kp = W::km(L, v, J), kq = W::km(L, v, J + 1);
    uint32_t fp, fq, rq, tp;
    if constexpr (W::per_lane || W::vgpr_k)
        asm volatile(DPOW_PIPE_BODY
                     : [pa] "+&v"(x[R::a][J]), [qb] "=&v"(x[R::b][J + 1]), [tq] "+v"(tq), [fp] "=&v"(fp),
                       [fq] "=&v"(fq), [rq] "=&v"(rq), [tp] "=&v"(tp)
                     : [pb] "v"(x[R::b][J]), [pc] "v"(x[R::c][J]), [pd] "v"(x[R::d][J]), [qc] "v"(x[R::c][J + 1]),
                       [qd] "v"(x[R::d][J + 1]), [qa] "v"(x[R::a][J + 1]), [kp] "v"(kp), [kq] "v"(kq),
                       [tt] "i"(tt<I>()), [sp] "i"(32 - md5_shift(I)), [sq] "i"(32 - md5_shift(I - 1)));
    else
        asm volatile(DPOW_PIPE_BODY
                     : [pa] "+&v"(x[R::a][J]), [qb] "=&v"(x[R::b][J + 1]), [tq] "+v"(tq), [fp] "=&v"(fp),
                       [fq] "=&v"(fq), [rq] "=&v"(rq), [tp] "=&v"(tp)
                     : [pb] "v"(x[R::b][J]), [pc] "v"(x[R::c][J]), [pd] "v"(x[R::d][J]), [qc] "v"(x[R::c][J + 1]),
                       [qd] "v"(x[R::d][J + 1]), [qa] "v"(x[R::a][J + 1]), [kp] "s"(kp), [kq] "s"(kq),
                       [tt] "i"(tt<I>()), [sp] "i"(32 - md5_shift(I)), [sq] "i"(32 - md5_shift(I - 1)));
}

template <int NBLK, int W0, int SH, int BLK, int I0, int J, class V>
DPOW_DEV void prologue(uint32_t (&x)[4][kNC], uint32_t &tq, const Launch &L, const V &v) {
    using R = Roles<I0>;
    using W = StepWord<NBLK, W0, SH, BLK, I0, V::kSpan>;
    const uint32_t kp = W::km(L, v, J), kq = W::km(L, v, J + 1);
    uint32_t fp, fq, tp;
    if constexpr (W::per_lane || W::vgpr_k)
        asm volatile(DPOW_PIPE_PRO
                     : [pa] "+&v"(x[R::a][J]), [tq] "=&v"(tq), [fp] "=&v"(fp), [fq] "=&v"(fq), [tp] "=&v"(tp)
                     : [pb] "v"(x[R::b][J]), [pc] "v"(x[R::c][J]), [pd] "v"(x[R::d][J]), [qb] "v"(x[R::b][J + 1]),
                       [qc] "v"(x[R::c][J + 1]), [qd] "v"(x[R::d][J + 1]), [qa] "v"(x[R::a][J + 1]), [kp] "v"(kp),
                       [kq] "v"(kq), [tt] "i"(tt<I0>()), [sp] "i"(32 - md5_shift(I0)));
    else
        asm volatile(DPOW_PIPE_PRO
                     : [pa] "+&v"(x[R::a][J]), [tq] "=&v"(tq), [fp] "=&v"(fp), [fq] "=&v"(fq), [tp] "=&v"(tp)
                     : [pb] "v"(x[R::b][J]), [pc] "v"(x[R::c][J]), [pd] "v"(x[R::d][J]), [qb] "v"(x[R::b][J + 1]),
                       [qc] "v"(x[R::c][J + 1]), [qd] "v"(x[R::d][J + 1]), [qa] "v"(x[R::a][J + 1]), [kp] "s"(kp),
                       [kq] "s"(kq), [tt] "i"(tt<I0>()), [sp] "i"(32 - md5_shift(I0)));
}

constexpr int kPairs = kNC / 2;

template <int NBLK, int W0, int SH, int BLK, int I, int IE, class V>
DPOW_DEV void run(uint32_t (&x)[4][kNC], uint32_t (&tq)[kPairs], const Launch &L, const V &v) {
    if constexpr (I < IE) {
        body<NBLK, W0, SH, BLK, I, 0>(x, tq[0], L, v);
        if constexpr (kPairs > 1) body<NBLK, W0, SH, BLK, I, 2>(x, tq[1], L, v);
        run<NBLK, W0, SH, BLK, I + 1, IE>(x, tq, L, v);
    }
}

template <int NBLK, int W0, int SH, int BLK, int I0, int IE, class V>
DPOW_DEV void steps(uint32_t (&x)[4][kNC], const Launch &L, const V &v) {
    static_assert(kNC == 2 || kNC == 4, "the pipelined path runs one or two candidate pairs");
    if constexpr (I0 < IE) {
        uint32_t tq[kPairs];
        prologue<NBLK, W0, SH, BLK, I0, 0>(x, tq[0], L, v);
        if constexpr (kPairs > 1) prologue<NBLK, W0, SH, BLK, I0, 2>(x, tq[1], L, v);
        run<NBLK, W0, SH, BLK, I0 + 1, IE>(x, tq, L, v);
        using E = Roles<IE - 1>;
#pragma unroll
        for (int p = 0; p < kPairs; ++p)
            x[E::a][2 * p + 1] = x[E::b][2 * p + 1] + __builtin_rotateleft32(tq[p], md5_shift(IE - 1));
    }
}

#undef DPOW_PIPE_BODY
#undef DPOW_PIPE_PRO
#undef DPOW_PAD_R
#undef DPOW_PAD_A

}

template <int NBLK, int W0, int SH, int NCAND, bool ONLY_D = false, bool RAW_D = false, class V>
DPOW_DEV void md5_tail(uint32_t (&out)[4][kNC], const Launch &L, const V &v) {
    static_assert(!RAW_D || (ONLY_D && NBLK == 1), "RAW_D: D word of one final block");
    uint32_t x[4][kNC];
#pragma unroll
    for (int j = 0; j < NCAND; ++j) {
        x[0][j] = L.iv[0]; x[1][j] = L.iv[1]; x[2][j] = L.iv[2]; x[3][j] = L.iv[3];
    }
    constexpr bool kPipe = NCAND == kNC && (kNC == 2 || kNC == 4);
    constexpr int kEnd0 = (ONLY_D && NBLK == 1) ? 62 : 64;
    constexpr int kLead = VgprK<NBLK, W0, SH, V::kSpan>::kLead;
    constexpr int kI0 = kPipe ? (W0 + kLead < kEnd0 ? W0 + kLead : kEnd0) : kEnd0;
    md5_steps<NBLK, W0, SH, 0, 0, kI0, NCAND>(x, L, v);
    if constexpr (kPipe) pipe::steps<NBLK, W0, SH, 0, kI0, kEnd0>(x, L, v);
#pragma unroll
    for (int j = 0; j < NCAND; ++j)
#pragma unroll
        for (int w = 0; w < 4; ++w) out[w][j] = (RAW_D && w == 3) ? x[w][j] : L.iv[w] + x[w][j];
    if constexpr (NBLK == 2) {
        constexpr int kEnd1 = ONLY_D ? 62 : 64;
#pragma unroll
        for (int j = 0; j < NCAND; ++j)
#pragma unroll
            for (int w = 0; w < 4; ++w) x[w][j] = out[w][j];
        if constexpr (kPipe)
            pipe::steps<NBLK, W0, SH, 1, 0, kEnd1>(x, L, v);
        else
            md5_steps<NBLK, W0, SH, 1, 0, kEnd1, NCAND>(x, L, v);
#pragma unroll
        for (int j = 0; j < NCAND; ++j)
#pragma unroll
            for (int w = 0; w < 4; ++w) out[w][j] += x[w][j];
    }
}

template <int SH, class V>
DPOW_DEV void var_words(V &v, int j, uint32_t vs, uint32_t loff, uint32_t d1) {
    v.lo_s[j] = vs << (8 * SH);
    v.lo_v = loff << (8 * SH);
    if constexpr (SH != 0) {
        v.hi_s[j] = (vs >> (32 - 8 * SH)) + d1;
        v.lane_k = SH == 3 && V::kSpan ? loff >> 8 : 0u;
    } else {
        v.hi_s[j] = 0u;
        v.lane_k = 0u;
    }
}

template <int NBLK, int W0, int SH, bool KS>
DPOW_DEV bool full_check(const Launch &L, const KConst &kc, uint32_t vs, uint32_t loff, const uint32_t (&sd)[3]) {
    VarWords<KS> v;
    v.kc = &kc;
    v.seg_d[0] = sd[0];
    v.seg_d[1] = sd[1];
    v.seg_d[2] = sd[2];
    var_words<SH>(v, 0, vs, loff, v.seg_d[0]);
    uint32_t out[4][kNC];
    md5_tail<NBLK, W0, SH, 1>(out, L, v);
    return trailing_zero_nibbles(out[0][0], out[1][0], out[2][0], out[3][0]) >= L.ntz;
}

__device__ __attribute__((noinline)) void publish(Ctrl *ctrl, Snap *snap, uint32_t seq, unsigned long long *claim,
                                                  Ctrl *ctrl_next) {
    if (ctrl_next == nullptr) {
        constexpr uintptr_t kRingBytes = kCtrlRing * kCtrlStride * sizeof(Ctrl);
        const uintptr_t a = reinterpret_cast<uintptr_t>(ctrl);
        ctrl_next =
            reinterpret_cast<Ctrl *>((a & ~(kRingBytes - 1)) | ((a + kCtrlStride * sizeof(Ctrl)) & (kRingBytes - 1)));
    }
    const unsigned long long t_start = __hip_atomic_load(&claim[1], __ATOMIC_RELAXED, __HIP_MEMORY_SCOPE_AGENT);
    for (uint32_t x = 0; x < kClaimCounters; ++x) claim[x * kClaimStride] = 0ull;
    claim[1] = 0ull;
    ctrl_next->best = kNoHit;
    ctrl_next->stop = 0u;
    ctrl_next->done = 0u;
    const unsigned long long best = __hip_atomic_load(&ctrl->best, __ATOMIC_RELAXED, __HIP_MEMORY_SCOPE_AGENT);
    const uint32_t stop = __hip_atomic_load(&ctrl->stop, __ATOMIC_RELAXED, __HIP_MEMORY_SCOPE_AGENT);
    __hip_atomic_store(&snap->best, best, __ATOMIC_RELAXED, __HIP_MEMORY_SCOPE_SYSTEM);
    __hip_atomic_store(&snap->stop, stop, __ATOMIC_RELAXED, __HIP_MEMORY_SCOPE_SYSTEM);
    __hip_atomic_store(&snap->t_start, t_start, __ATOMIC_RELAXED, __HIP_MEMORY_SCOPE_SYSTEM);
    __hip_atomic_store(&snap->t_end, __builtin_amdgcn_s_memrealtime(), __ATOMIC_RELAXED, __HIP_MEMORY_SCOPE_SYSTEM);
    __hip_atomic_store(&snap->seq, seq, __ATOMIC_RELEASE, __HIP_MEMORY_SCOPE_SYSTEM);
#if DPOW_WAVE_TRACE
    g_wave_trace[kTraceFields * (kTraceWaves - 2) + 3] = __builtin_amdgcn_s_memrealtime();
#endif
}

constexpr int kPad4B = 63;
DPOW_DEV void watcher(const Launch &L) {
    if (threadIdx.x != 0) return;
    __hip_atomic_store(&L.claim[1], __builtin_amdgcn_s_memrealtime(), __ATOMIC_RELAXED, __HIP_MEMORY_SCOPE_AGENT);
    unsigned long long node_seen = ~0ull, bound_seen = L.bound0, early_seen = kNoHit;
#if DPOW_WAVE_TRACE
    unsigned long long *wt = g_wave_trace + kTraceFields * (kTraceWaves - 1);
    wt[0] = __builtin_amdgcn_s_memrealtime();
    wt[1] = wt[2] = 0;
#endif
    for (;;) {
        const unsigned long long *const nbp = L.node_best ? L.node_best : L.ext_bound;
        const uint32_t *const nsp = L.node_stop ? L.node_stop : L.cancel;
        const uint32_t done = __hip_atomic_load(&L.ctrl->done, __ATOMIC_RELAXED, __HIP_MEMORY_SCOPE_AGENT);
        const unsigned long long b = __hip_atomic_load(&L.ctrl->best, __ATOMIC_RELAXED, __HIP_MEMORY_SCOPE_AGENT);
        const uint32_t stale = __hip_atomic_load(L.stale, __ATOMIC_RELAXED, __HIP_MEMORY_SCOPE_SYSTEM);
        const uint32_t cancel = __hip_atomic_load(L.cancel, __ATOMIC_RELAXED, __HIP_MEMORY_SCOPE_SYSTEM);
        const unsigned long long eb = __hip_atomic_load(L.ext_bound, __ATOMIC_RELAXED, __HIP_MEMORY_SCOPE_SYSTEM);
        const unsigned long long nb = __hip_atomic_load(nbp, __ATOMIC_RELAXED, __HIP_MEMORY_SCOPE_SYSTEM);
        const uint32_t nstop = __hip_atomic_load(nsp, __ATOMIC_RELAXED, __HIP_MEMORY_SCOPE_SYSTEM);
        if (done >= L.done_target) {
#if DPOW_WAVE_TRACE
            wt[3] = __builtin_amdgcn_s_memrealtime();
#endif
            return;
        }
        if (L.early && b < early_seen) {
#if DPOW_WAVE_TRACE
            if (wt[2] == 0) wt[2] = __builtin_amdgcn_s_memrealtime();
#endif
            early_seen = b;
            __hip_atomic_store(L.early, b, __ATOMIC_RELAXED, __HIP_MEMORY_SCOPE_SYSTEM);
        }
        bool stop = cancel != 0u || (int32_t)(stale - L.seq) >= 0;
        if (eb < bound_seen) {
            bound_seen = eb;
            __hip_atomic_fetch_min(&L.ctrl->best, eb, __ATOMIC_RELAXED, __HIP_MEMORY_SCOPE_AGENT);
        }
        if (L.node_best) {
            if (nb < node_seen) {
#if DPOW_WAVE_TRACE
                if (wt[1] == 0 && nb < kNoHit) wt[1] = __builtin_amdgcn_s_memrealtime();
#endif
                node_seen = nb;
                __hip_atomic_fetch_min(&L.ctrl->best, nb, __ATOMIC_RELAXED, __HIP_MEMORY_SCOPE_AGENT);
            }
            stop = stop || nstop != 0u;
        }
        if (stop) {
            __hip_atomic_store(&L.ctrl->stop, 1u, __ATOMIC_RELAXED, __HIP_MEMORY_SCOPE_AGENT);
            return;
        }
        __builtin_amdgcn_s_sleep(kWatchSleep);
    }
}

template <bool kOpaque>
DPOW_DEV unsigned long long claim_issue(unsigned long long *ctr, uint32_t lane) {
    unsigned long long v = 0;
    if constexpr (kOpaque) {
        uint32_t z;
        asm volatile("v_mov_b32 %0, 0" : "=v"(z));
        ctr += z;
    }
    if (lane == 0) v = __hip_atomic_fetch_add(ctr, 1ull, __ATOMIC_RELAXED, __HIP_MEMORY_SCOPE_AGENT);
    return v;
}

DPOW_DEV uint64_t claim_take(unsigned long long v, uint32_t x, uint64_t base) {
    const uint32_t lo = __builtin_amdgcn_readfirstlane((uint32_t)v);
    const uint32_t hi = __builtin_amdgcn_readfirstlane((uint32_t)(v >> 32));
    return (((uint64_t)hi << 32) | lo) * kClaimCounters + x + base;
}

DPOW_DEV uint64_t claim_next(unsigned long long *ctr, uint32_t x, uint32_t lane, uint64_t base) {
    return claim_take(claim_issue<false>(ctr, lane), x, base);
}

DPOW_DEV uint64_t lane_range_mask(int64_t lo, int64_t hi) {
    lo = lo < 0 ? 0 : (lo > 64 ? 64 : lo);
    hi = hi < 0 ? 0 : (hi > 64 ? 64 : hi);
    if (hi <= lo) return 0;
    const uint64_t upto_hi = hi == 64 ? ~0ull : ((1ull << hi) - 1ull);
    const uint64_t below_lo = lo == 64 ? ~0ull : ((1ull << lo) - 1ull);
    return upto_hi & ~below_lo;
}

constexpr uint64_t kNoHitG = ~0ull;

template <int NBLK, int W0, int SH, bool EQ, bool KSPAN>
DPOW_DEV uint64_t hash_wave_block(const Launch &L, const KConst &kc, uint64_t i0, uint32_t lane, uint32_t loff) {
    static_assert(!EQ || NBLK == 1, "the D-equality test needs one final block");
    static_assert(KSPAN || SH == 3, "only the SH = 3 kernels have a narrow (R >= 64) instantiation");
    uint32_t vs[kNC];
    VarWords<KSPAN> v;
    v.kc = &kc;
    v.seg_d[0] = v.seg_d[1] = v.seg_d[2] = 0u;
    uint32_t d1 = 0u;
    if constexpr (SH != 0) {
        uint32_t d2;
        seg_deltas<W0, SH>(L, (uint32_t)((i0 >> L.rbits) >> 24), d1, d2);
    }
#pragma unroll
    for (int j = 0; j < kNC; ++j) {
        vs[j] = wave_uniform_v(i0 + 64u * j, L.rbits, L.base_tb);
        var_words<SH>(v, j, vs[j], loff, d1);
    }
    uint32_t dig[4][kNC];
    md5_tail<NBLK, W0, SH, kNC, true, EQ>(dig, L, v);

    uint64_t bal[kNC];
    uint64_t any = 0;
#pragma unroll
    for (int j = 0; j < kNC; ++j) {
        bal[j] = EQ ? __ballot(dig[3][j] == L.deq) : __ballot(dig[3][j] <= L.dle);
        any |= bal[j];
    }
    if (any != 0) {
#pragma unroll
        for (int j = 0; j < kNC; ++j) {
            const uint64_t ij = i0 + 64u * j;
            uint64_t m = bal[j] & lane_range_mask((int64_t)(L.i_begin - ij), (int64_t)(L.i_end - ij));
            if (!EQ && m != 0) m &= __ballot((dig[3][j] & L.dmask) == 0u);
            if (m != 0 && L.ntz > 8u) {
                uint32_t d0, sd[3];
                seg_all_deltas<NBLK, W0, SH>(L, seg_id((ij < L.i_begin ? L.i_begin : ij) >> L.rbits), d0, sd);
                const bool ok = ((m >> lane) & 1ull) && full_check<NBLK, W0, SH, KSPAN>(L, kc, vs[j], loff, sd);
                m = __ballot(ok);
            }
            if (m != 0) {
                const uint64_t g = global_of_local(ij + (uint64_t)__builtin_ctzll(m), L.rbits, L.base_tb);
                if (lane == 0) {
                    const unsigned long long prev = __hip_atomic_fetch_min(
                        &L.ctrl->best, (unsigned long long)g, __ATOMIC_RELAXED, __HIP_MEMORY_SCOPE_AGENT);
                    asm volatile("; dpow: atomicMin performed (%0)" ::"v"(prev));
                }
                return g;
            }
        }
    }
    return kNoHitG;
}

template <int NBLK, int W0>
constexpr bool kLongSgpr = NBLK == 2 || W0 >= kSgprLongW0;
template <int NBLK, int W0, int SH>
constexpr bool kW15Sgpr = (NBLK == 2 && W0 == 15) || (NBLK == 2 && SH == 3 && (W0 == 13 || W0 == 14)) ||
                          (NBLK == 1 && W0 == 11 && SH == 3);

template <int NBLK, int W0, int SH>
constexpr bool kLaunchPoll = NBLK == 1 || SH == 1 || SH == 2 || (SH == 0 && W0 == 15) || (SH == 3 && W0 >= 14);

template <int NBLK, int W0>
constexpr int kNarrowPoll = DPOW_NPOLL >= 0 ? DPOW_NPOLL : narrow_knobs(NBLK, W0).poll;
template <int NBLK, int W0>
constexpr int kNarrowSgpr = DPOW_NSGPR > 0 ? DPOW_NSGPR : narrow_knobs(NBLK, W0).sgpr;
template <int NBLK, int W0, int SH, bool KS>
constexpr bool kPollOf = SH == 3 && !KS && kNarrowPoll<NBLK, W0> >= 0 ? kNarrowPoll<NBLK, W0> != 0
                                                                     : kLaunchPoll<NBLK, W0, SH>;
template <int NBLK, int W0, int SH, bool KS>
constexpr bool kShort96 = NBLK == 1 && !DPOW_VLS && KS && W0 < kSgprLongW0 &&
                          (SH == 1 || SH == 2 || (SH == 0 && (W0 == 3 || W0 >= 5)) ||
                           (SH == 3 && ((W0 >= 2 && W0 <= 5) || W0 == 7)));
template <int NBLK, int W0, int SH, bool KS>
constexpr int kSgprOf = SH == 3 && !KS && kNarrowSgpr<NBLK, W0> > 0 ? kNarrowSgpr<NBLK, W0>
                        : kW15Sgpr<NBLK, W0, SH> ? 2 : kLongSgpr<NBLK, W0> || kShort96<NBLK, W0, SH, KS> ? 1 : 0;

template <int NBLK, int W0, int SH, bool EQ, bool KSPAN>
DPOW_DEV void search_body(const Launch &L) {
    if (blockIdx.x == 0) {
        watcher(L);
        return;
    }
#if DPOW_WAVE_TRACE
    const unsigned long long t_start = __builtin_amdgcn_s_memrealtime();
    unsigned long long t_first = 0, n_wb = 0, t_last = 0, c_last = 0, reason = 0, t_hit = 0;
#endif
    if constexpr (EQ && NBLK == 1 && W0 == 1 && SH == 0 && !DPOW_VLS)
        asm volatile(".rept %0\n s_nop 0\n .endr" ::"i"(kPad4B));
    const uint32_t lane = threadIdx.x & 63u;
    const uint32_t loff = lane_offset(L.rbits, lane);
    KConst kc;
    kconst_init<NBLK, W0, SH, 0, 0, KSPAN>(kc, L);
    uint32_t cur_seg_v;
    asm("v_mov_b32 %0, %1" : "=v"(cur_seg_v) : "s"(L.seg0));
    uint32_t lov = loff;

    unsigned long long best = __hip_atomic_load(&L.ctrl->best, __ATOMIC_RELAXED, __HIP_MEMORY_SCOPE_AGENT);
    best = best < L.bound0 ? best : L.bound0;
    uint32_t stop = __hip_atomic_load(&L.ctrl->stop, __ATOMIC_RELAXED, __HIP_MEMORY_SCOPE_AGENT);

    __builtin_amdgcn_s_setprio(1);
    constexpr bool kDeferClaims = NBLK == 1;
    uint32_t x = (blockIdx.x - 1u) % kClaimCounters;
    const bool skip = stop != 0u || global_of_local(L.i_begin, L.rbits, L.base_tb) >= best;
    const uint64_t cbase = kStaticFirst ? L.n_static : 0;
    uint64_t claim;
    if constexpr (kStaticFirst) {
        const uint32_t wave_id =
            __builtin_amdgcn_readfirstlane((blockIdx.x - 1u) * (kBlockThreads / 64) + threadIdx.x / 64u);
        claim = skip ? L.n_chunks
                     : (wave_id < cbase ? (uint64_t)wave_id : claim_next(L.claim + x * kClaimStride, x, lane, cbase));
    } else {
        claim = skip ? L.n_chunks : claim_next(L.claim + x * kClaimStride, x, lane, cbase);
    }
#if DPOW_WAVE_TRACE
    t_first = __builtin_amdgcn_s_memrealtime() + (claim & 0);
#endif
    uint32_t hops = 0;
    for (;;) {
        if (claim >= L.n_chunks) {
#if DPOW_WAVE_TRACE
            reason = 1;
#endif
            if (skip || ++hops >= kClaimCounters) break;
            x = (x + 1u) % kClaimCounters;
            const unsigned long long seen =
                __hip_atomic_load(L.claim + x * kClaimStride, __ATOMIC_RELAXED, __HIP_MEMORY_SCOPE_AGENT);
            claim = seen * kClaimCounters + x + cbase < L.n_chunks
                        ? claim_next(L.claim + x * kClaimStride, x, lane, cbase)
                        : L.n_chunks;
            continue;
        }
        unsigned long long next_v = 0;
        uint64_t next = 0;
        bool issued = false;
        if constexpr (kDeferClaims) (void)issued;
        else next = claim_next(L.claim + x * kClaimStride, x, lane, cbase);
        const bool big = claim < L.n_big;
        if (!big) __builtin_amdgcn_s_setprio(0);
        const uint64_t b_begin = big ? claim * L.chunk : L.n_big * L.chunk + (claim - L.n_big) * L.chunk_tail;
        const uint32_t csz = big ? L.chunk : L.chunk_tail;
        const uint32_t nb = (uint32_t)(b_begin + csz < L.n_wblocks ? csz : L.n_wblocks - b_begin);
        const uint64_t i_first = L.wb_begin + b_begin * (uint64_t)kWaveBlock;
        if (stop != 0u ||
            global_of_local(i_first < L.i_begin ? L.i_begin : i_first, L.rbits, L.base_tb) >= best) {
#if DPOW_WAVE_TRACE
            reason = stop != 0u ? 3 : 2;
#endif
            break;
        }
#if DPOW_WAVE_TRACE
        t_last = __builtin_amdgcn_s_memrealtime();
        c_last = claim;
#endif
        uint64_t i0 = i_first;
        uint32_t left = nb;
        const uint32_t poll_wb = kPollOf<NBLK, W0, SH, KSPAN> ? L.poll_wb : (uint32_t)DPOW_POLL_WB;
        for (;;) {
            uint32_t q = left < poll_wb ? left : poll_wb;
            {
                const uint32_t sg = seg_id((i0 < L.i_begin ? L.i_begin : i0) >> L.rbits);
                if (sg != __builtin_amdgcn_readfirstlane(cur_seg_v)) {
                    asm volatile("v_mov_b32 %0, %1" : "=v"(cur_seg_v) : "s"(sg));
                    uint32_t d0, d[3];
                    seg_all_deltas<NBLK, W0, SH>(L, sg, d0, d);
                    kconst_seg<NBLK, W0, SH, 0, 0, KSPAN>(kc, L, d);
                    if constexpr (SH == 0) lov = lane_offset(L.rbits, lane) + d0;
                }
            }
            left -= q;
            if constexpr (kDeferClaims) {
                if (left == 0) {
                    next_v = claim_issue<true>(L.claim + x * kClaimStride, lane);
                    issued = true;
                }
            }
            const unsigned long long best_seen =
                __hip_atomic_load(&L.ctrl->best, __ATOMIC_RELAXED, __HIP_MEMORY_SCOPE_AGENT);
            const uint32_t stop_seen = __hip_atomic_load(&L.ctrl->stop, __ATOMIC_RELAXED, __HIP_MEMORY_SCOPE_AGENT);
            bool hit = false;
            for (; q != 0; --q, i0 += (uint64_t)kWaveBlock) {
#if DPOW_WAVE_TRACE
                ++n_wb;
#endif
                const uint64_t g = hash_wave_block<NBLK, W0, SH, EQ, KSPAN>(L, kc, i0, lane, SH == 0 ? lov : loff);
                if (g != kNoHitG) {
                    best = g < best ? g : best;
                    hit = true;
#if DPOW_WAVE_TRACE
                    if (t_hit == 0) t_hit = __builtin_amdgcn_s_memrealtime();
#endif
                    break;
                }
            }
            best = best_seen < best ? best_seen : best;
            stop = stop_seen;
            if (hit || left == 0 || stop != 0u || global_of_local(i0, L.rbits, L.base_tb) >= best) break;
        }
        if constexpr (kDeferClaims) {
            if (!issued) {
#if DPOW_WAVE_TRACE
                reason = 4;
#endif
                break;
            }
            claim = claim_take(next_v, x, cbase);
        } else {
            claim = next;
        }
    }
#if DPOW_WAVE_TRACE
    const uint32_t wave = (blockIdx.x - 1u) * (kBlockThreads / 64) + threadIdx.x / 64u;
    if (lane == 0 && wave < kTraceWaves) {
        unsigned long long *w = g_wave_trace + kTraceFields * wave;
        w[0] = t_start;
        w[1] = t_first;
        w[2] = __builtin_amdgcn_s_memrealtime();
        w[3] = n_wb;
        w[4] = t_last;
        w[5] = c_last;
        w[6] = reason;
        w[7] = t_hit;
    }
#endif
    if constexpr (kDeferClaims) {
        asm volatile("s_waitcnt vmcnt(0)" ::: "memory");
    }
#if DPOW_WAVE_TRACE
    const unsigned long long t_claims = __builtin_amdgcn_s_memrealtime();
#endif
    __builtin_amdgcn_fence(__ATOMIC_RELEASE, "workgroup");
    __syncthreads();
    if (threadIdx.x == 0) {
#if DPOW_WAVE_TRACE
        const unsigned long long t_bar = __builtin_amdgcn_s_memrealtime();
#endif
        if constexpr (kXcdRetire) {
            const uint32_t n_wg = gridDim.x - 1u;
            const uint32_t xr = (blockIdx.x - 1u) % kClaimCounters;
            const uint32_t nx = n_wg / kClaimCounters + (xr < n_wg % kClaimCounters ? 1u : 0u);
            unsigned long long *const xc = L.claim + xr * kClaimStride + 2;
            const unsigned long long px = __hip_atomic_fetch_add(xc, 1ull, __ATOMIC_RELAXED, __HIP_MEMORY_SCOPE_AGENT);
            if (px + 1ull == (unsigned long long)nx) {
                __hip_atomic_store(xc, 0ull, __ATOMIC_RELAXED, __HIP_MEMORY_SCOPE_AGENT);
                const uint32_t prev = __hip_atomic_fetch_add(&L.ctrl->done, nx, __ATOMIC_RELAXED, __HIP_MEMORY_SCOPE_AGENT);
#if DPOW_WAVE_TRACE
                if (prev + nx == L.done_target) {
                    unsigned long long *r = g_wave_trace + kTraceFields * (kTraceWaves - 2);
                    r[0] = t_claims;
                    r[1] = t_bar;
                    r[2] = __builtin_amdgcn_s_memrealtime() + (prev & 0);
                }
#endif
                if (prev + nx == L.done_target)
                    publish(L.ctrl, L.snap, L.seq, L.claim, kPollOf<NBLK, W0, SH, KSPAN> ? L.ctrl_next : nullptr);
            }
        } else {
            const uint32_t prev = __hip_atomic_fetch_add(&L.ctrl->done, 1u, __ATOMIC_RELAXED, __HIP_MEMORY_SCOPE_AGENT);
#if DPOW_WAVE_TRACE
            if (prev + 1u == L.done_target) {
                unsigned long long *r = g_wave_trace + kTraceFields * (kTraceWaves - 2);
                r[0] = t_claims;
                r[1] = t_bar;
                r[2] = __builtin_amdgcn_s_memrealtime() + (prev & 0);
            }
#endif
            if (prev + 1u == L.done_target) publish(L.ctrl, L.snap, L.seq, L.claim, kPollOf<NBLK, W0, SH, KSPAN> ? L.ctrl_next : nullptr);
        }
    }
}

template <int NBLK, int W0, int SH, bool EQ, bool KSPAN>
__global__ void __launch_bounds__(kBlockThreads) __attribute__((amdgpu_num_sgpr(DPOW_NUM_SGPR)))
md5_search_kernel(const Launch L) {
    search_body<NBLK, W0, SH, EQ, KSPAN>(L);
}

template <int NBLK, int W0, int SH, bool EQ, bool KSPAN>
__global__ void __launch_bounds__(kBlockThreads) __attribute__((amdgpu_num_sgpr(DPOW_NUM_SGPR_LONG)))
md5_search_kernel_lsgpr(const Launch L) {
    search_body<NBLK, W0, SH, EQ, KSPAN>(L);
}

template <int NBLK, int W0, int SH, bool EQ, bool KSPAN>
__global__ void __launch_bounds__(kBlockThreads) __attribute__((amdgpu_num_sgpr(DPOW_NUM_SGPR_W15)))
md5_search_kernel_w15sgpr(const Launch L) {
    search_body<NBLK, W0, SH, EQ, KSPAN>(L);
}

}
}
```

### distributed-proof-of-work_amd/csrc/md5_variant.hip

```cpp
#include "md5_search_kernel.h"
#include "md5_variants.h"

#include <hip/hip_ext.h>

#ifndef DPOW_VNBLK
#error "DPOW_VNBLK must be defined"
#endif
#ifndef DPOW_VSH
#error "DPOW_VSH must be defined"
#endif

namespace dpow {

namespace {
using namespace DPOW_KNS;
using KernelFn = void (*)(Launch);
template <int NBLK, int W0, int SH, bool EQ, bool KSPAN>
constexpr KernelFn kernel_of() {
    if constexpr (kSgprOf<NBLK, W0, SH, KSPAN> == 2) return md5_search_kernel_w15sgpr<NBLK, W0, SH, EQ, KSPAN>;
    else if constexpr (kSgprOf<NBLK, W0, SH, KSPAN> == 1) return md5_search_kernel_lsgpr<NBLK, W0, SH, EQ, KSPAN>;
    else return md5_search_kernel<NBLK, W0, SH, EQ, KSPAN>;
}
#define DPOW_K(w, e, nar) \
    kernel_of<DPOW_VNBLK, w, DPOW_VSH, e, !(DPOW_VSH == 3 && nar && narrow_knobs(DPOW_VNBLK, w).on)>()
#if DPOW_VNBLK == 1
constexpr int kW0Lo = 0;
#define DPOW_ROW(e, n)                                                                                              \
    {DPOW_K(0, e, n), DPOW_K(1, e, n), DPOW_K(2, e, n),  DPOW_K(3, e, n),  DPOW_K(4, e, n),  DPOW_K(5, e, n),        \
     DPOW_K(6, e, n), DPOW_K(7, e, n), DPOW_K(8, e, n),  DPOW_K(9, e, n),  DPOW_K(10, e, n), DPOW_K(11, e, n),       \
     DPOW_K(12, e, n), DPOW_K(13, e, n)}
const KernelFn kTable[2][2][14] = {{DPOW_ROW(false, false), DPOW_ROW(false, true)},
                                   {DPOW_ROW(true, false), DPOW_ROW(true, true)}};
#else
constexpr int kW0Lo = 12;
#define DPOW_ROW(e, n) {DPOW_K(12, e, n), DPOW_K(13, e, n), DPOW_K(14, e, n), DPOW_K(15, e, n)}
const KernelFn kTable[2][2][4] = {{DPOW_ROW(false, false), DPOW_ROW(false, true)},
                                  {DPOW_ROW(false, false), DPOW_ROW(false, true)}};
#endif
#undef DPOW_ROW
#undef DPOW_K
constexpr int kW0N = sizeof(kTable[0][0]) / sizeof(kTable[0][0][0]);

KernelFn pick(int w0, bool eq, bool narrow) {
    return (w0 >= kW0Lo && w0 < kW0Lo + kW0N) ? kTable[eq ? 1 : 0][narrow ? 1 : 0][w0 - kW0Lo] : nullptr;
}
}

#if DPOW_VLS
#define DPOW_SFX _ls
#else
#define DPOW_SFX
#endif
#define DPOW_CAT4(a, b, c, d) a##b##_##c##d
#define DPOW_NAME2(a, b, c, d) DPOW_CAT4(a, b, c, d)
#define DPOW_NAME(a, b, c) DPOW_NAME2(a, b, c, DPOW_SFX)

hipError_t DPOW_NAME(variant_launch_, DPOW_VNBLK, DPOW_VSH)(int w0, const Launch &L, uint32_t grid,
                                                           hipStream_t stream) {
    KernelFn fn = pick(w0, use_d_equality(DPOW_VNBLK, L.ntz), L.rbits >= 6u);
    if (!fn) return hipErrorInvalidValue;
    hipLaunchKernelGGL(fn, dim3(grid), dim3(kBlockThreads), 0, stream, L);
    return hipGetLastError();
}

hipError_t DPOW_NAME(variant_prepare_, DPOW_VNBLK, DPOW_VSH)() {
    for (const auto &eq : kTable)
        for (const auto &row : eq)
            for (KernelFn fn : row) {
                hipFuncAttributes a;
                const hipError_t e = hipFuncGetAttributes(&a, reinterpret_cast<const void *>(fn));
                if (e != hipSuccess) return e;
            }
    return hipSuccess;
}

hipError_t DPOW_NAME(variant_occupancy_, DPOW_VNBLK, DPOW_VSH)(int w0, int *blocks_per_cu) {
    KernelFn fn = pick(w0, false, true);
    if (!fn) return hipErrorInvalidValue;
    return hipOccupancyMaxActiveBlocksPerMultiprocessor(blocks_per_cu, reinterpret_cast<const void *>(fn),
                                                        kBlockThreads, 0);
}

}

#if DPOW_WAVE_TRACE && DPOW_VNBLK == 1 && DPOW_VSH == 0
#if DPOW_VLS
extern "C" int dpow_diag_wave_trace_ls(unsigned long long *out, size_t n) {
#else
extern "C" int dpow_diag_wave_trace(unsigned long long *out, size_t n) {
#endif
    if (n > dpow::DPOW_KNS::kTraceWaves * dpow::DPOW_KNS::kTraceFields)
        n = dpow::DPOW_KNS::kTraceWaves * dpow::DPOW_KNS::kTraceFields;
    return hipMemcpyFromSymbol(out, HIP_SYMBOL(dpow::DPOW_KNS::g_wave_trace), n * 8, 0, hipMemcpyDeviceToHost) == hipSuccess
               ? 0
               : -2;
}
#endif
```

### distributed-proof-of-work_amd/csrc/md5_variants.h

```cpp
#pragma once
#include <hip/hip_runtime.h>

#include "dpow_common.h"

namespace dpow {

#define DPOW_DECL_VARIANT(n, s)                                                                  \
    hipError_t variant_launch_##n##_##s(int w0, const Launch &L, uint32_t grid, hipStream_t st); \
    hipError_t variant_occupancy_##n##_##s(int w0, int *blocks_per_cu);                        \
    hipError_t variant_prepare_##n##_##s();
DPOW_DECL_VARIANT(1, 0)
DPOW_DECL_VARIANT(1, 1)
DPOW_DECL_VARIANT(1, 2)
DPOW_DECL_VARIANT(1, 3)
DPOW_DECL_VARIANT(2, 0)
DPOW_DECL_VARIANT(2, 1)
DPOW_DECL_VARIANT(2, 2)
DPOW_DECL_VARIANT(2, 3)
DPOW_DECL_VARIANT(1, 0_ls)
DPOW_DECL_VARIANT(2, 0_ls)
#undef DPOW_DECL_VARIANT

inline bool variant_exists(int nblk, int w0, int sh) {
    if (sh < 0 || sh > 3) return false;
    if (nblk == 1) return w0 >= 0 && w0 <= 13;
    if (nblk == 2) return w0 >= 12 && w0 <= 15;
    return false;
}

hipError_t search_launch(int nblk, int w0, int sh, const Launch &L, uint32_t grid, hipStream_t stream);
hipError_t search_occupancy(int nblk, int w0, int sh, int *blocks_per_cu);
hipError_t search_prepare();

struct StartK0 {
    uint32_t r;
    uint32_t base_tb;
    uint32_t nblk;
    uint32_t p;
    uint32_t ntz;
    uint32_t seq;
    Snap *snap;
    uint32_t iv[4];
    uint32_t T[32];
};
hipError_t search_k0(const StartK0 &k0, hipStream_t stream);
hipError_t search_k0_prepare();
hipError_t context_init(Ctrl *ctrl, uint32_t n_ctrl, unsigned long long *claims, uint32_t n_claims,
                        hipStream_t stream);
hipError_t clock_probe(unsigned long long *out, hipStream_t stream);

}
```

### distributed-proof-of-work_amd/csrc/plan.cpp

```cpp
#include "plan.h"

#include <algorithm>

#include <string.h>

#include "md5_host.h"

namespace dpow {

uint32_t chunk_len_of(uint64_t k) {
    uint32_t n = 0;
    while (k) { ++n; k >>= 8; }
    return n;
}

uint64_t segment_end(uint64_t k) {
    const uint32_t L = chunk_len_of(k);
    if (L == 0) return 1;
    return 1ull << (8 * L);
}

uint64_t word2_period(uint32_t sh) {
    return (sh == 1 || sh == 2) ? 1ull << (56 - 8 * sh) : 0;
}

uint32_t remainder_bits(uint32_t worker_bits) { return 8u - (worker_bits % 9u); }

uint32_t base_thread_byte(uint32_t worker_byte, uint32_t worker_bits) {
    return (uint32_t)((worker_byte << remainder_bits(worker_bits)) & 0xFFu);
}

int WindowPlanner::init(const uint8_t *nonce, size_t nonce_len, uint32_t ntz, uint32_t worker_byte,
                        uint32_t worker_bits, uint64_t k_begin, uint64_t k_end) {
    if (nonce_len && !nonce) return -1;
    if (worker_byte > 255u) return -1;
    if (k_end > DPOW_K_LIMIT) return DPOW_ERANGE;
    nonce_ = nonce;
    nonce_len_ = nonce_len;
    ntz_ = ntz;
    rbits_ = remainder_bits(worker_bits);
    base_tb_ = base_thread_byte(worker_byte, worker_bits);
    blk_v_ = nonce_len / 64;
    p_ = (uint32_t)(nonce_len % 64);
    k_ = k_begin;
    k_end_ = k_end;
    lspan_end_ = lspan_end(nonce_len, rbits_, ntz);
    for (int w = 0; w < 4; ++w) iv_[w] = kMd5IV[w];
    for (size_t b = 0; b < blk_v_; ++b) {
        uint32_t M[16];
        for (int w = 0; w < 16; ++w) M[w] = load_le32(nonce + 64 * b + 4 * w);
        md5_compress(iv_, M);
    }
    return 0;
}

uint32_t WindowPlanner::nblk_of(uint32_t chunk_len) const {
    const size_t msg_len = nonce_len_ + 1 + chunk_len;
    return (uint32_t)((msg_len + 8) / 64 + 1 - blk_v_);
}

void WindowPlanner::build_template(uint64_t k, uint32_t L, uint32_t nblk, uint32_t T[32]) const {
    uint8_t buf[128];
    memset(buf, 0, sizeof buf);
    const uint32_t p = p_;
    if (p) memcpy(buf, nonce_ + 64 * blk_v_, p);
    for (uint32_t j = 3; j < L; ++j) buf[p + 1 + j] = (uint8_t)(k >> (8 * j));
    buf[p + 1 + L] = 0x80;
    const uint64_t bits = (uint64_t)(nonce_len_ + 1 + L) * 8u;
    for (int j = 0; j < 8; ++j) buf[64 * nblk - 8 + j] = (uint8_t)(bits >> (8 * j));
    for (uint32_t w = 0; w < 32; ++w) T[w] = w < 16 * nblk ? load_le32(buf + 4 * w) : 0u;
}

uint64_t lspan_end(size_t nonce_len, uint32_t rbits, uint32_t ntz) {
    if (!(nonce_len % 4 == 0 && rbits >= 1)) return 0;
    return expected_first_hit(ntz, rbits) <= kLspanMaxExpect ? 1ull << 24 : 1ull << 16;
}

bool WindowPlanner::lseg_template(uint64_t k) const {
    return k < lspan_end_;
}

bool WindowPlanner::next(PlannedLaunch &pl) {
    if (k_ >= k_end_) return false;
    const uint64_t k = k_;
    memset(&pl, 0, sizeof pl);
    Launch &Lh = pl.L;
    const uint32_t p = p_;
    const uint64_t R = 1ull << rbits_;
    uint64_t ke = segment_end(k) < k_end_ ? segment_end(k) : k_end_;
    if (const uint64_t w2 = word2_period(p_ % 4)) {
        const uint64_t we = (k / w2 + 1) * w2;
        if (we < ke) ke = we;
    }
    const uint64_t cap_end = cap_k_ && k_end_ - k > cap_k_ ? k + cap_k_ : k_end_;
    cap_k_ = 0;
    if (cap_end < ke) ke = cap_end;
    const uint32_t L = chunk_len_of(k);
    const uint32_t nblk = nblk_of(L);
    pl.k0 = k == 0;
    uint32_t L_last = L;
    if (!pl.k0 && k >= 1 && lseg_template(k)) {
        uint64_t e = ke;
        while (e < k_end_ && e < lspan_end_ && nblk_of(chunk_len_of(e)) == nblk &&
               (segment_end(e) < k_end_ ? segment_end(e) : k_end_) <= cap_end) {
            e = segment_end(e) < k_end_ ? segment_end(e) : k_end_;
            L_last = chunk_len_of(e - 1);
        }
        if (e > ke) {
            ke = e;
            Lh.lspan = 1;
        }
    }
    build_template(k, L, nblk, Lh.T);
    for (int w = 0; w < 4; ++w) Lh.iv[w] = iv_[w];
    if (lseg_template(k)) {
        uint32_t d0, d1, dlen;
        lseg_deltas(L, d0, d1, dlen);
        const uint32_t w0 = p / 4, lenw = 16 * nblk - 2;
        if (w0 + 1 == lenw) {
            dlen += d1;
            d1 = 0;
        }
        Lh.T[w0] -= d0;
        Lh.T[w0 + 1] -= d1;
        Lh.T[lenw] -= dlen;
    }
    for (uint32_t b = 0; b < nblk; ++b)
        for (int s = 0; s < 64; ++s) Lh.KT[64 * b + s] = kMd5K[s] + Lh.T[16 * b + md5_word(s)];
    Lh.i_begin = k << rbits_;
    Lh.i_end = pl.k0 ? R : ke << rbits_;
    Lh.wb_begin = Lh.i_begin & ~(uint64_t)(kWaveBlock - 1);
    Lh.n_wblocks = (Lh.i_end - Lh.wb_begin + (uint64_t)kWaveBlock - 1) / (uint64_t)kWaveBlock;
    Lh.rbits = rbits_;
    Lh.base_tb = base_tb_;
    Lh.dmask = tail_nibble_mask(ntz_ < 8 ? ntz_ : 8);
    Lh.dle = tail_prefilter_le(ntz_);
    Lh.deq = 0u - iv_[3];
    Lh.ntz = ntz_;
    Lh.seg_first = (uint32_t)(k >> 24);
    Lh.seg0 = lseg_template(k) ? kLsegBase : seg_id(k);
    if (pl.k0) ke = 1;
    pl.info.k_begin = k;
    pl.info.k_end = ke;
    pl.info.i_begin = Lh.i_begin;
    pl.info.i_end = Lh.i_end;
    pl.info.nblk = nblk;
    pl.info.w0 = p / 4;
    pl.info.sh = p % 4;
    pl.info.chunk_len = L;
    pl.info.chunk_len_last = L_last;
    pl.info.start_kernel = pl.k0 ? 1u : 0u;
    k_ = ke;
    return true;
}

int plan_window(const uint8_t *nonce, size_t nonce_len, uint32_t ntz, uint32_t worker_byte,
                uint32_t worker_bits, uint64_t k_begin, uint64_t k_end, std::vector<PlannedLaunch> &out) {
    out.clear();
    WindowPlanner wp;
    int rc = wp.init(nonce, nonce_len, ntz, worker_byte, worker_bits, k_begin, k_end);
    if (rc < 0) return rc;
    PlannedLaunch pl;
    while (wp.next(pl)) out.push_back(pl);
    return (int)out.size();
}

void candidate_words(const PlannedLaunch &pl, uint64_t local_idx, uint32_t words[32]) {
    const Launch &Lh = pl.L;
    for (uint32_t w = 0; w < 16 * pl.info.nblk; ++w) words[w] = Lh.T[w];
    const uint64_t i0 = local_idx & ~63ull;
    const uint32_t lane = (uint32_t)(local_idx & 63u);
    const uint32_t V = wave_uniform_v(i0, Lh.rbits, Lh.base_tb) + lane_offset(Lh.rbits, lane);
    const uint32_t sh = pl.info.sh, w0 = pl.info.w0;
    words[w0] += V << (8 * sh);
    if (sh) words[w0 + 1] += V >> (32 - 8 * sh);
    if (Lh.seg0 == kLsegBase && !pl.k0) {
        uint32_t d0, d1, dlen;
        lseg_deltas(chunk_len_of(local_idx >> Lh.rbits), d0, d1, dlen);
        const uint32_t lenw = 16 * pl.info.nblk - 2;
        if (w0 + 1 == lenw) {
            dlen += d1;
            d1 = 0;
        }
        words[w0] += d0;
        words[w0 + 1] += d1;
        words[lenw] += dlen;
    }
    {
        uint32_t d1, d2;
        const uint32_t seg = (uint32_t)((local_idx >> Lh.rbits) >> 24);
        seg_word_deltas(Lh.T[w0 + 1], Lh.T[w0 + 2], seg, Lh.seg_first, sh, d1, d2);
        words[w0 + 1] += d1;
        if (sh == 3 && w0 + 2 != 16 * pl.info.nblk - 2) words[w0 + 2] += d2;
    }
}

uint64_t expected_first_hit(uint32_t ntz, uint32_t rbits) {
    if (ntz >= 14) return ~0ull;
    return ((1ull << (4 * ntz)) << rbits) >> 8;
}

int size_launch(PlannedLaunch &pl, uint64_t max_blocks, uint64_t expect, uint64_t *worker_blocks_out,
                uint64_t min_chunk, uint64_t claims_per_wave) {
    Launch &L = pl.L;
    constexpr uint64_t wpb = kBlockThreads / 64;
    uint64_t worker_blocks = (L.n_wblocks + wpb - 1) / wpb;
    if (worker_blocks > max_blocks) worker_blocks = max_blocks;
    uint64_t span_wb = L.n_wblocks;
    if (expect / (uint64_t)kWaveBlock < span_wb) span_wb = expect / (uint64_t)kWaveBlock;
    uint64_t chunk = span_wb / (worker_blocks * wpb * claims_per_wave);
    if (chunk < min_chunk) chunk = min_chunk;
    if (chunk > kMaxChunk) chunk = kMaxChunk;
    if ((pl.info.k_begin >> 24) != ((pl.info.k_end - 1) >> 24) || L.lspan) {
        while (chunk & (chunk - 1)) chunk &= chunk - 1;
        if (L.lspan && chunk > (2ull << L.rbits)) chunk = 2ull << L.rbits;
        L.wb_begin = L.i_begin & ~(chunk * (uint64_t)kWaveBlock - 1);
        L.n_wblocks = (L.i_end - L.wb_begin + (uint64_t)kWaveBlock - 1) / (uint64_t)kWaveBlock;
        worker_blocks = (L.n_wblocks + wpb - 1) / wpb;
        if (worker_blocks > max_blocks) worker_blocks = max_blocks;
    }
    const uint64_t chunk_tail = kTailChunk < chunk ? kTailChunk : chunk;
    const uint64_t tail_wb = worker_blocks * wpb * kTailClaimsPerWave * chunk_tail;
    const uint64_t n_big = L.n_wblocks > tail_wb ? (L.n_wblocks - tail_wb) / chunk : 0;
    const uint64_t rest = L.n_wblocks - n_big * chunk;
    const uint64_t n_chunks = n_big + (rest + chunk_tail - 1) / chunk_tail;
    uint64_t need_blocks = (n_chunks + wpb - 1) / wpb;
    if (need_blocks < n_chunks && need_blocks < kClaimCounters)
        need_blocks = n_chunks < kClaimCounters ? n_chunks : kClaimCounters;
    if (worker_blocks > need_blocks) worker_blocks = need_blocks;
    const uint64_t min_blocks = n_chunks < kClaimCounters ? n_chunks : kClaimCounters;
    if (worker_blocks < min_blocks && min_blocks <= max_blocks) worker_blocks = min_blocks;
    if (worker_blocks < kClaimCounters && worker_blocks < n_chunks) return DPOW_EINVAL;
    L.chunk = (uint32_t)chunk;
    L.chunk_tail = (uint32_t)chunk_tail;
    L.n_big = n_big;
    L.n_chunks = n_chunks;
    L.n_head = 2 * worker_blocks * wpb;
    L.n_static = L.seg0 == kLsegBase && !pl.k0
                     ? (n_chunks < worker_blocks * wpb ? n_chunks : worker_blocks * wpb)
                     : 0;
    *worker_blocks_out = worker_blocks;
    return 0;
}

uint32_t launch_poll_wb(uint32_t ntz, uint32_t rbits) {
    const uint32_t slow = DPOW_POLL_WB > 0 ? DPOW_POLL_WB : 16;
    const uint64_t expect = expected_first_hit(ntz, rbits);
    if (expect <= kTinyExpect) return 1;
    if (expect <= kNearExpect) return kNearPollWb;
    if (expect <= kMidExpect) return kMidPollWb;
    return expect <= kFastPollCands ? kFastPollWb : slow;
}

uint64_t launch_claims_per_wave(uint32_t ntz, uint32_t rbits) {
    return expected_first_hit(ntz, rbits) <= kFastPollCands ? kShortClaimsPerWave : kClaimsPerWave;
}

uint64_t launch_min_chunk(uint32_t ntz, uint32_t rbits) {
    const uint64_t expect = expected_first_hit(ntz, rbits);
    if (expect <= kTinyExpect) return kTinyChunk;
    return expect > kMidChunkExpect && expect <= kMidExpect ? kMidChunk : kMinChunk;
}

int size_search_launch(PlannedLaunch &pl, uint32_t ntz, uint64_t cus, uint64_t share, const LaunchKnobs &knobs,
                       uint64_t *worker_blocks, uint64_t active) {
    Launch &L = pl.L;
    share = std::max<uint64_t>(share, 1);
    active = std::max<uint64_t>(active, share);
    const uint64_t bpc = knobs.bpc ? knobs.bpc : launch_blocks_per_cu(L.i_end - L.i_begin, ntz, L.rbits, active);
    const uint64_t max_blocks = std::max<uint64_t>(cus * bpc / share, kClaimCounters);
    const int rc = size_launch(pl, max_blocks, expected_first_hit(ntz, L.rbits), worker_blocks,
                               knobs.min_chunk ? knobs.min_chunk : launch_min_chunk(ntz, L.rbits),
                               knobs.cpw ? knobs.cpw : launch_claims_per_wave(ntz, L.rbits));
    if (rc < 0) return rc;
    L.poll_wb = knobs.poll_wb ? knobs.poll_wb : launch_poll_wb(ntz, L.rbits);
    return 0;
}

uint64_t grid_share(uint64_t active, const LaunchKnobs &knobs) {
    const uint64_t cap = knobs.share_max ? knobs.share_max : kShareMax;
    return std::max<uint64_t>(1, std::min(active, cap));
}

bool cap_shared_launch(WindowPlanner &planner, PlannedLaunch &pl, uint64_t active, const LaunchKnobs &knobs) {
    if (active <= 1 || pl.k0) return false;
    const double ns = knobs.share_launch_us ? knobs.share_launch_us * 1e3 : (double)kShareLaunchNs;
    const uint64_t cap_k = std::max<uint64_t>(1, (uint64_t)(kEstRate / (double)active * ns * 1e-9) >> pl.L.rbits);
    if (pl.info.k_end - pl.info.k_begin <= cap_k) return false;
    planner.restart(pl.info.k_begin, cap_k);
    planner.next(pl);
    return true;
}

uint64_t launch_blocks_per_cu(uint64_t candidates, uint32_t ntz, uint32_t rbits, uint64_t share) {
    const auto dev = [share](uint64_t v) { return share > 1 && v > ~0ull / share ? ~0ull : v * (share ? share : 1); };
    const uint64_t expect = dev(expected_first_hit(ntz, rbits));
    const uint64_t eff = dev(candidates) < expect ? dev(candidates) : expect;
    if (expect <= kTinyExpect || dev(candidates) <= kTinyLaunch) return kMaxBlocksPerCu < 2 ? kMaxBlocksPerCu : 2;
    if (eff <= (1ull << 22)) return kMaxBlocksPerCu < 3 ? kMaxBlocksPerCu : 3;
    if (eff <= kMidExpect) return kMaxBlocksPerCu < 4 ? kMaxBlocksPerCu : 4;
    if (kFiveExpect && expect <= kFiveExpect) return kMaxBlocksPerCu < 5 ? kMaxBlocksPerCu : 5;
    return kMaxBlocksPerCu;
}

}
```

### distributed-proof-of-work_amd/csrc/plan.h

```cpp
#pragma once
#include <stddef.h>
#include <stdint.h>

#include <vector>

#include "../../include/dpow.h"
#include "dpow_common.h"

namespace dpow {

struct PlannedLaunch {
    dpow_plan_launch info;
    Launch L;
    bool k0 = false;
};

uint32_t chunk_len_of(uint64_t k);
uint64_t segment_end(uint64_t k);
uint64_t word2_period(uint32_t sh);
constexpr uint64_t kLspanMaxExpect = 1ull << 28;
uint64_t lspan_end(size_t nonce_len, uint32_t rbits, uint32_t ntz);
uint32_t remainder_bits(uint32_t worker_bits);
uint32_t base_thread_byte(uint32_t worker_byte, uint32_t worker_bits);

class WindowPlanner {
   public:
    int init(const uint8_t *nonce, size_t nonce_len, uint32_t ntz, uint32_t worker_byte, uint32_t worker_bits,
             uint64_t k_begin, uint64_t k_end);
    bool next(PlannedLaunch &out);
    void restart(uint64_t k, uint64_t max_k) {
        k_ = k;
        cap_k_ = max_k;
    }

   private:
    uint32_t nblk_of(uint32_t chunk_len) const;
    bool lseg_template(uint64_t k) const;
    void build_template(uint64_t k, uint32_t chunk_len, uint32_t nblk, uint32_t T[32]) const;
    const uint8_t *nonce_ = nullptr;
    size_t nonce_len_ = 0, blk_v_ = 0;
    uint32_t p_ = 0, ntz_ = 0, rbits_ = 0, base_tb_ = 0;
    uint64_t k_ = 0, k_end_ = 0;
    uint64_t cap_k_ = 0;
    uint64_t lspan_end_ = 0;
    uint32_t iv_[4] = {0, 0, 0, 0};
};

int plan_window(const uint8_t *nonce, size_t nonce_len, uint32_t ntz, uint32_t worker_byte,
                uint32_t worker_bits, uint64_t k_begin, uint64_t k_end, std::vector<PlannedLaunch> &out);

void candidate_words(const PlannedLaunch &pl, uint64_t local_idx, uint32_t words[32]);

constexpr uint64_t kClaimsPerWave = 16;
constexpr uint64_t kMinChunk = 4;
#ifndef DPOW_MAX_CHUNK
#define DPOW_MAX_CHUNK 32
#endif
constexpr uint64_t kMaxChunk = DPOW_MAX_CHUNK;
#ifndef DPOW_TAIL_CLAIMS
#define DPOW_TAIL_CLAIMS 2
#endif
constexpr uint64_t kTailClaimsPerWave = DPOW_TAIL_CLAIMS;
#ifndef DPOW_TAIL_CHUNK
#define DPOW_TAIL_CHUNK 4
#endif
constexpr uint64_t kTailChunk = DPOW_TAIL_CHUNK;
static_assert((kMinChunk & (kMinChunk - 1)) == 0 && (kMaxChunk & (kMaxChunk - 1)) == 0 &&
                  (kTailChunk & (kTailChunk - 1)) == 0 && kTailChunk <= kMinChunk,
              "chunk bounds are powers of two (segment alignment)");
int size_launch(PlannedLaunch &pl, uint64_t max_blocks, uint64_t expect, uint64_t *worker_blocks,
                uint64_t min_chunk = kMinChunk, uint64_t claims_per_wave = kClaimsPerWave);
uint64_t expected_first_hit(uint32_t ntz, uint32_t rbits);

#ifndef DPOW_POLL_WB
#define DPOW_POLL_WB 16
#endif
#ifndef DPOW_FAST_POLL_WB
#define DPOW_FAST_POLL_WB 8
#endif
#ifndef DPOW_MID_POLL_WB
#define DPOW_MID_POLL_WB 4
#endif
#ifndef DPOW_NEAR_POLL_WB
#define DPOW_NEAR_POLL_WB 2
#endif
constexpr uint64_t kNearExpect = 1ull << 24;
constexpr uint32_t kFastPollWb = DPOW_FAST_POLL_WB;
constexpr uint32_t kMidPollWb = DPOW_MID_POLL_WB;
constexpr uint32_t kNearPollWb = DPOW_NEAR_POLL_WB;
constexpr uint64_t kFastPollCands = 1ull << 30;
uint32_t launch_poll_wb(uint32_t ntz, uint32_t rbits);
#ifndef DPOW_TINY_EXPECT_LOG2
#define DPOW_TINY_EXPECT_LOG2 23
#endif
constexpr uint64_t kTinyExpect = 1ull << DPOW_TINY_EXPECT_LOG2;
constexpr uint64_t kTinyLaunch = 1ull << 21;
constexpr uint64_t kMidExpect = 1ull << 26;
#ifndef DPOW_FIVE_EXPECT_LOG2
#define DPOW_FIVE_EXPECT_LOG2 31
#endif
constexpr uint64_t kFiveExpect = DPOW_FIVE_EXPECT_LOG2 ? 1ull << DPOW_FIVE_EXPECT_LOG2 : 0;
constexpr uint64_t kTinyChunk = 2;
#ifndef DPOW_MID_CHUNK
#define DPOW_MID_CHUNK 8
#endif
constexpr uint64_t kMidChunk = DPOW_MID_CHUNK;
constexpr uint64_t kMidChunkExpect = 1ull << 24;
uint64_t launch_min_chunk(uint32_t ntz, uint32_t rbits);
constexpr uint64_t kShortClaimsPerWave = 64;
uint64_t launch_claims_per_wave(uint32_t ntz, uint32_t rbits);

#ifndef DPOW_BLOCKS_PER_CU
#define DPOW_BLOCKS_PER_CU 6
#endif
constexpr uint64_t kMaxBlocksPerCu = DPOW_BLOCKS_PER_CU;
uint64_t launch_blocks_per_cu(uint64_t candidates, uint32_t ntz, uint32_t rbits, uint64_t share = 1);

struct LaunchKnobs {
    uint32_t bpc = 0, min_chunk = 0, cpw = 0, poll_wb = 0;
    uint32_t share_launch_us = 0;
    uint32_t share_max = 0;
};
int size_search_launch(PlannedLaunch &pl, uint32_t ntz, uint64_t cus, uint64_t share, const LaunchKnobs &knobs,
                       uint64_t *worker_blocks, uint64_t active = 1);

#ifndef DPOW_SHARE_MAX
#define DPOW_SHARE_MAX 2
#endif
#ifndef DPOW_SHARE_LAUNCH_US
#define DPOW_SHARE_LAUNCH_US 8000
#endif
constexpr uint64_t kShareMax = DPOW_SHARE_MAX;
#ifndef DPOW_YOUNG_US
#define DPOW_YOUNG_US 2000
#endif
constexpr int64_t kYoungNs = (int64_t)DPOW_YOUNG_US * 1000;
constexpr int64_t kRecentNs = 100 * 1000 * 1000;
constexpr int64_t kShareLaunchNs = (int64_t)DPOW_SHARE_LAUNCH_US * 1000;
constexpr double kEstRate = 2.3e11;
uint64_t grid_share(uint64_t active, const LaunchKnobs &knobs);
bool cap_shared_launch(WindowPlanner &planner, PlannedLaunch &pl, uint64_t active, const LaunchKnobs &knobs);

}
```

### include/dpow_diag.h

```cpp
#ifndef DPOW_DIAG_H
#define DPOW_DIAG_H

#ifdef __cplusplus
extern "C" {
#endif

int dpow_diag_valu_rate(int device, int kind, double *lane_ops_per_s, double *clock_ghz);

int dpow_diag_launch_latency(int device, int mode, int reps, double *median_us);

int dpow_diag_dword_test(const uint8_t *nonce, size_t nonce_len, uint32_t ntz, uint64_t k,
                         uint32_t iv_d, uint32_t state_d);

typedef struct dpow_diag_launch {
    uint64_t k_begin, k_end;
    uint64_t i_begin, i_end;
    uint64_t wb_begin;
    uint64_t n_wblocks;
    uint64_t n_big, n_chunks;
    uint64_t worker_blocks;
    uint32_t chunk, chunk_tail;
    uint32_t rbits;
    uint32_t wave_block;
    uint64_t n_static;
    uint32_t poll_wb;
    uint32_t pad;
} dpow_diag_launch;
int dpow_diag_launch_geometry(const uint8_t *nonce, size_t nonce_len, uint32_t ntz, uint32_t worker_byte,
                              uint32_t worker_bits, uint64_t k_begin, uint64_t k_end, uint32_t cus,
                              uint32_t share, dpow_diag_launch *out, size_t max_launches);

uint64_t dpow_diag_blocks_per_cu(uint64_t candidates, uint32_t ntz, uint32_t worker_bits);

int dpow_diag_search_times(struct dpow_ctx *ctx, int64_t out[8]);

typedef struct dpow_diag_launch_time {
    uint64_t seq;
    int32_t kind;
    int32_t recorded;
    int64_t queued_ns, seen_ns;
    uint64_t t_start_tick, t_end_tick;
    uint64_t candidates, g_end;
    uint64_t best;
} dpow_diag_launch_time;
int dpow_diag_search_launches(struct dpow_ctx *ctx, int64_t *t0_ns, dpow_diag_launch_time *out,
                              size_t max_launches);

int dpow_diag_clock_sync(struct dpow_ctx *ctx, int reps, int64_t *offset_ns);

int dpow_diag_vote_latency(uint32_t world, int reps, double *last_us, double *all_us);

int dpow_diag_node_post_at(struct dpow_node_slot *slot, uint64_t global_idx, int64_t t_ns);

int dpow_diag_node_alias(struct dpow_ctx *ctx, void **cached, void **lookup);


#ifdef __cplusplus
}
#endif
#endif
```

Baseline: 218.8 GH/s.

## Add segment-inner MD5 kernel that reuses per-wave prefix across 2^24 segments

Adds a new kernel variant (_si) for single-block layouts with w0<=3 and sh==0. Each wave computes the MD5 prefix steps up to W0+1 and the per-lane W0 round constants once, then iterates over several 2^24-candidate segments, redoing only the steps from W0+1 onward. The launch planner cuts windows to a bounded segment count and resizes chunks per segment. This aims to amortise the prefix and per-candidate setup over many segments, at the cost of extra VGPRs (w0km array), a changed pipeline lead, and more complex index mapping for hit reporting.

```diff
diff --git a/distributed-proof-of-work_amd/csrc/dpow_api.cpp b/distributed-proof-of-work_amd/csrc/dpow_api.cpp
--- a/distributed-proof-of-work_amd/csrc/dpow_api.cpp
+++ b/distributed-proof-of-work_amd/csrc/dpow_api.cpp
@@ -472,8 +472,10 @@
         }
         const uint64_t share = grid_share(active, c->knobs);
         cap_shared_launch(planner, pl, active, c->knobs);
+        const bool seg_inner = seg_inner_select(planner, pl, ntz, c->knobs.seg_inner);
         uint64_t worker_blocks = 0;
         rc = size_search_launch(pl, ntz, c->cus, share, c->knobs, &worker_blocks, active);
+        if (rc >= 0 && seg_inner) rc = seg_inner_size(pl, worker_blocks, &worker_blocks);
         if (rc < 0) return set_error(rc, "dpow_search: launch grid leaves a claim counter without waves");
         done_target += (uint32_t)worker_blocks;
         L.claim = c->d_claims + (li % kClaimRing) * kClaimSlot;
@@ -493,7 +495,7 @@
                           c->stream);
         if (e != hipSuccess) return hip_fail(e, "search_launch");
         if (!md5_queued) c->diag_t[1] = now_ns() - sw.t0;
-        diag_queued(li, seq, 1, L.i_end - L.i_begin, pl.info.k_end << 8);
+        diag_queued(li, seq, L.n_seg != 0u ? 2 : 1, L.i_end - L.i_begin, pl.info.k_end << 8);
         md5_queued = true;
         slot.seq = seq;
         slot.in_flight = true;
@@ -641,6 +643,7 @@
     if (const char *pw = getenv("DPOW_DIAG_CPW")) c->knobs.cpw = (uint32_t)std::max(0, atoi(pw));
     if (const char *pw = getenv("DPOW_DIAG_SHARE_LAUNCH_US")) c->knobs.share_launch_us = (uint32_t)std::max(0, atoi(pw));
     if (const char *pw = getenv("DPOW_DIAG_SHARE_MAX")) c->knobs.share_max = (uint32_t)std::max(0, atoi(pw));
+    if (const char *pw = getenv("DPOW_DIAG_SEG_INNER")) c->knobs.seg_inner = atoi(pw) != 0 ? 1 : 0;
     if (const char *pw = getenv("DPOW_DIAG_MIN_CHUNK")) {
         const uint32_t v = (uint32_t)std::max(0, atoi(pw));
         if (v && !(v & (v - 1))) c->knobs.min_chunk = v;
@@ -1169,22 +1172,35 @@
     return 0;
 }
 
-int dpow_diag_launch_geometry(const uint8_t *nonce, size_t nonce_len, uint32_t ntz, uint32_t worker_byte,
-                              uint32_t worker_bits, uint64_t k_begin, uint64_t k_end, uint32_t cus, uint32_t share,
-                              dpow_diag_launch *out, size_t max_launches) {
-    if (cus == 0 || share == 0) return set_error(DPOW_EINVAL, "dpow_diag_launch_geometry: cus and share must be > 0");
+namespace {
+int launch_geometry(const char *who, const uint8_t *nonce, size_t nonce_len, uint32_t ntz, uint32_t worker_byte,
+                    uint32_t worker_bits, uint64_t k_begin, uint64_t k_end, uint32_t cus, uint32_t share,
+                    int seg_inner_mode, bool recut, dpow_diag_launch *out, size_t max_launches) {
+    if (cus == 0 || share == 0) return set_error(DPOW_EINVAL, who);
     WindowPlanner planner;
     const int rc = planner.init(nonce, nonce_len, ntz, worker_byte, worker_bits, k_begin, k_end);
-    if (rc < 0) return set_error(rc, "dpow_diag_launch_geometry: bad arguments");
+    if (rc < 0) return set_error(rc, who);
     PlannedLaunch pl;
     size_t n = 0;
     const LaunchKnobs policy{};
     while (planner.next(pl)) {
         if (pl.k0) continue;
         cap_shared_launch(planner, pl, share, policy);
+        const bool seg_inner = seg_inner_select(planner, pl, ntz, seg_inner_mode);
         uint64_t wblocks = 0;
-        const int r = size_search_launch(pl, ntz, cus, grid_share(share, policy), policy, &wblocks, share);
-        if (r < 0) return set_error(r, "dpow_diag_launch_geometry: launch grid leaves a claim counter without waves");
+        int r = size_search_launch(pl, ntz, cus, grid_share(share, policy), policy, &wblocks, share);
+        uint32_t n_seg = 0;
+        if (r >= 0 && seg_inner) {
+            PlannedLaunch cut = pl;
+            uint64_t wb2 = wblocks;
+            r = seg_inner_size(cut, wblocks, &wb2);
+            n_seg = cut.L.n_seg;
+            if (recut) {
+                pl = cut;
+                wblocks = wb2;
+            }
+        }
+        if (r < 0) return set_error(r, who);
         if (out && n < max_launches) {
             dpow_diag_launch &d = out[n];
             d.k_begin = pl.info.k_begin;
@@ -1202,10 +1218,54 @@
             d.wave_block = kWaveBlock;
             d.n_static = pl.L.n_static;
             d.poll_wb = pl.L.poll_wb;
+            d.n_seg = n_seg;
         }
         ++n;
     }
     return (int)n;
+}
+}
+
+int dpow_diag_launch_geometry(const uint8_t *nonce, size_t nonce_len, uint32_t ntz, uint32_t worker_byte,
+                              uint32_t worker_bits, uint64_t k_begin, uint64_t k_end, uint32_t cus, uint32_t share,
+                              dpow_diag_launch *out, size_t max_launches) {
+    return launch_geometry("dpow_diag_launch_geometry: bad arguments or grid", nonce, nonce_len, ntz, worker_byte,
+                           worker_bits, k_begin, k_end, cus, share, -1, false, out, max_launches);
+}
+
+int dpow_diag_seg_inner_geometry(const uint8_t *nonce, size_t nonce_len, uint32_t ntz, uint32_t worker_byte,
+                                 uint32_t worker_bits, uint64_t k_begin, uint64_t k_end, uint32_t cus, int mode,
+                                 dpow_diag_launch *out, size_t max_launches) {
+    return launch_geometry("dpow_diag_seg_inner_geometry: bad arguments or grid", nonce, nonce_len, ntz,
+                           worker_byte, worker_bits, k_begin, k_end, cus, 1, mode, true, out, max_launches);
+}
+
+int dpow_diag_seg_inner_candidate(const uint8_t *nonce, size_t nonce_len, uint32_t ntz, uint32_t worker_byte,
+                                  uint32_t worker_bits, uint64_t k_begin, uint64_t k_end, int mode,
+                                  uint64_t local_idx, uint32_t iv_out[4], uint32_t words_out[32],
+                                  uint32_t *nblk_out) {
+    if (!iv_out || !words_out || !nblk_out)
+        return set_error(DPOW_EINVAL, "dpow_diag_seg_inner_candidate: NULL argument");
+    WindowPlanner planner;
+    const int rc = planner.init(nonce, nonce_len, ntz, worker_byte, worker_bits, k_begin, k_end);
+    if (rc < 0) return set_error(rc, "dpow_diag_seg_inner_candidate: bad arguments");
+    PlannedLaunch pl;
+    const LaunchKnobs policy{};
+    while (planner.next(pl)) {
+        if (pl.k0) continue;
+        const bool seg_inner = seg_inner_select(planner, pl, ntz, mode);
+        if (local_idx < pl.L.i_begin || local_idx >= pl.L.i_end) continue;
+        uint64_t wblocks = 0;
+        int r = size_search_launch(pl, ntz, 256, 1, policy, &wblocks, 1);
+        if (r >= 0 && seg_inner) r = seg_inner_size(pl, wblocks, &wblocks);
+        if (r < 0) return set_error(r, "dpow_diag_seg_inner_candidate: sizing failed");
+        for (int w = 0; w < 4; ++w) iv_out[w] = pl.L.iv[w];
+        memset(words_out, 0, 32 * sizeof(uint32_t));
+        candidate_words(pl, local_idx, words_out);
+        *nblk_out = pl.info.nblk;
+        return seg_inner ? 1 : 0;
+    }
+    return set_error(DPOW_EINVAL, "dpow_diag_seg_inner_candidate: index outside the window");
 }
 
 int dpow_diag_node_alias(dpow_ctx *c, void **cached, void **lookup) {
diff --git a/distributed-proof-of-work_amd/csrc/dpow_common.h b/distributed-proof-of-work_amd/csrc/dpow_common.h
--- a/distributed-proof-of-work_amd/csrc/dpow_common.h
+++ b/distributed-proof-of-work_amd/csrc/dpow_common.h
@@ -97,7 +97,7 @@
     uint64_t n_head;
     uint64_t n_static;
     uint32_t poll_wb;
-    uint32_t reserved0;
+    uint32_t n_seg;
     unsigned long long *claim;
     Ctrl *ctrl;
     Ctrl *ctrl_next;
@@ -141,6 +141,8 @@
     return e == 0 ? 0xFFFFFFFFu : e >= 8 ? 0u : (0xFFFFFFFFu >> (4 * e));
 }
 
+DPOW_HD bool seg_inner_layout(uint32_t nblk, uint32_t w0, uint32_t sh) { return nblk == 1 && sh == 0 && w0 <= 3; }
+
 DPOW_HD bool use_d_equality(uint32_t nblk, uint32_t ntz) { return nblk == 1 && ntz >= 8; }
 
 DPOW_HD uint32_t bswap32(uint32_t x) {
diff --git a/distributed-proof-of-work_amd/csrc/md5_dispatch.cpp b/distributed-proof-of-work_amd/csrc/md5_dispatch.cpp
--- a/distributed-proof-of-work_amd/csrc/md5_dispatch.cpp
+++ b/distributed-proof-of-work_amd/csrc/md5_dispatch.cpp
@@ -4,6 +4,11 @@
 
 hipError_t search_launch(int nblk, int w0, int sh, const Launch &L, uint32_t grid, hipStream_t stream) {
     if (!variant_exists(nblk, w0, sh)) return hipErrorInvalidValue;
+    if (L.n_seg != 0u) {
+        if (!seg_inner_exists(nblk, w0, sh) || !use_d_equality((uint32_t)nblk, L.ntz) || L.seg0 == kLsegBase)
+            return hipErrorInvalidValue;
+        return variant_launch_1_0_si(w0, L, grid, stream);
+    }
     if (L.seg0 == kLsegBase) {
         if (sh != 0) return hipErrorInvalidValue;
         return nblk == 1 ? variant_launch_1_0_ls(w0, L, grid, stream)
@@ -33,7 +38,7 @@
     if (e == hipSuccess) e = variant_prepare_##n##_##s();
     DPOW_PREP(1, 0) DPOW_PREP(1, 1) DPOW_PREP(1, 2) DPOW_PREP(1, 3)
     DPOW_PREP(2, 0) DPOW_PREP(2, 1) DPOW_PREP(2, 2) DPOW_PREP(2, 3)
-    DPOW_PREP(1, 0_ls) DPOW_PREP(2, 0_ls)
+    DPOW_PREP(1, 0_ls) DPOW_PREP(2, 0_ls) DPOW_PREP(1, 0_si)
 #undef DPOW_PREP
     return e;
 }
diff --git a/distributed-proof-of-work_amd/csrc/md5_search_kernel.h b/distributed-proof-of-work_amd/csrc/md5_search_kernel.h
--- a/distributed-proof-of-work_amd/csrc/md5_search_kernel.h
+++ b/distributed-proof-of-work_amd/csrc/md5_search_kernel.h
@@ -6,8 +6,25 @@
 #ifndef DPOW_VLS
 #define DPOW_VLS 0
 #endif
+#ifndef DPOW_VSI
+#define DPOW_VSI 0
+#endif
+#ifndef DPOW_SI_LEAD
+#define DPOW_SI_LEAD 5
+#endif
+#ifndef DPOW_SI_PAD
+#define DPOW_SI_PAD 0
+#endif
+#ifndef DPOW_SI_VSEG
+#define DPOW_SI_VSEG 1
+#endif
+#if DPOW_VLS && DPOW_VSI
+#error "DPOW_VLS and DPOW_VSI are separate units"
+#endif
 #if DPOW_VLS
 #define DPOW_KNS lsk
+#elif DPOW_VSI
+#define DPOW_KNS sik
 #else
 #define DPOW_KNS k
 #endif
@@ -145,16 +162,17 @@
 struct VgprK {
     static constexpr bool kNarrow = SH == 3 && !KS;
     static constexpr int kEnd0 = NBLK == 1 ? 62 : 64;
-    static constexpr int kLead = pipe_lead(NBLK, W0, SH, kNarrow);
+    static constexpr int kLead = DPOW_VSI && DPOW_SI_LEAD > 0 ? DPOW_SI_LEAD : pipe_lead(NBLK, W0, SH, kNarrow);
     static constexpr int kI0 = W0 + kLead < kEnd0 ? W0 + kLead : kEnd0;
     static constexpr bool run(int blk, int i) { return !(blk == NBLK - 1 && i >= 62); }
-    static constexpr bool seg(int blk, int i) { return seg_word<NBLK, W0, SH>(16 * blk + md5_word(i)) && run(blk, i); }
+    static constexpr bool segw(int blk, int i) { return seg_word<NBLK, W0, SH>(16 * blk + md5_word(i)) && run(blk, i); }
+    static constexpr bool seg(int blk, int i) { return (!DPOW_VSI || DPOW_SI_VSEG) && segw(blk, i); }
     static constexpr bool eligible(int blk, int i) {
         const int m = 16 * blk + md5_word(i);
         const bool zero = m > W0 + 2 && m != 16 * NBLK - 2;
         const bool lane = m == W0 || (SH != 0 && m == W0 + 1);
         const bool piped = blk > 0 || i >= kI0;
-        return !zero && !lane && piped && run(blk, i) && !seg(blk, i);
+        return !zero && !lane && piped && run(blk, i) && !segw(blk, i);
     }
     static constexpr int rank(int blk, int i) {
         int r = 0;
@@ -241,7 +259,16 @@
     uint32_t lane_k;
     const KConst *kc;
     uint32_t seg_d[3];
+#if DPOW_VSI
+    uint32_t w0km[4][kNC];
+#endif
 };
+
+constexpr int step_of_word(int r, int w) {
+    for (int i = 16 * r; i < 16 * r + 16; ++i)
+        if (md5_word(i) == w) return i;
+    return -1;
+}
 
 template <int NBLK, int W0, int SH, int BLK, int I, bool KS>
 struct StepWord {
@@ -253,7 +280,11 @@
     static DPOW_DEV uint32_t km(const Launch &L, const VarWords<KS> &v, int j) {
         uint32_t k = zero_word ? kMd5K[I] : vgpr_k ? v.kc->v[64 * BLK + I] : L.KT[64 * BLK + I];
         if constexpr (seg && !vgpr_k) k += seg_add<NBLK, W0>(m, v.seg_d);
+#if DPOW_VSI
+        if constexpr (m == W0) k = v.w0km[I / 16][j];
+#else
         if constexpr (m == W0) k = (k + v.lo_s[j]) + v.lo_v;
+#endif
         if constexpr (SH != 0 && m == W0 + 1) {
             k += v.hi_s[j];
             if constexpr (SH == 3 && KS) k += v.lane_k;
@@ -432,6 +463,18 @@
     }
 }
 
+#if DPOW_VSI
+template <int W0, class V>
+DPOW_DEV void w0km_fill(V &v, int j, const Launch &L) {
+    constexpr int i0 = step_of_word(0, W0), i1 = step_of_word(1, W0), i2 = step_of_word(2, W0),
+                  i3 = step_of_word(3, W0);
+    v.w0km[0][j] = (L.KT[i0] + v.lo_s[j]) + v.lo_v;
+    v.w0km[1][j] = (L.KT[i1] + v.lo_s[j]) + v.lo_v;
+    v.w0km[2][j] = (L.KT[i2] + v.lo_s[j]) + v.lo_v;
+    v.w0km[3][j] = (L.KT[i3] + v.lo_s[j]) + v.lo_v;
+}
+#endif
+
 template <int NBLK, int W0, int SH, bool KS>
 DPOW_DEV bool full_check(const Launch &L, const KConst &kc, uint32_t vs, uint32_t loff, const uint32_t (&sd)[3]) {
     VarWords<KS> v;
@@ -440,6 +483,9 @@
     v.seg_d[1] = sd[1];
     v.seg_d[2] = sd[2];
     var_words<SH>(v, 0, vs, loff, v.seg_d[0]);
+#if DPOW_VSI
+    w0km_fill<W0>(v, 0, L);
+#endif
     uint32_t out[4][kNC];
     md5_tail<NBLK, W0, SH, 1>(out, L, v);
     return trailing_zero_nibbles(out[0][0], out[1][0], out[2][0], out[3][0]) >= L.ntz;
@@ -833,23 +879,242 @@
     }
 }
 
+#if DPOW_VSI
+constexpr uint32_t kSegLimitNone = 0xFFFFFFFFu;
+
+DPOW_DEV uint64_t local_ceil_of_global(uint64_t g, uint32_t rbits, uint32_t base_tb) {
+    const uint64_t k = g >> 8;
+    const uint32_t tb = (uint32_t)(g & 0xFFu);
+    if (tb < base_tb) return k << rbits;
+    const uint32_t t = tb - base_tb;
+    return t >> rbits ? (k + 1u) << rbits : (k << rbits) + t;
+}
+
+struct SegLimit {
+    uint32_t q, r;
+};
+DPOW_DEV SegLimit seg_limit_of(const Launch &L, unsigned long long best) {
+    const uint32_t segbits = 24u + L.rbits;
+    const uint64_t ib = local_ceil_of_global(best, L.rbits, L.base_tb);
+    const uint64_t rel = ib > L.wb_begin ? ib - L.wb_begin : 0ull;
+    const uint64_t q = rel >> segbits;
+    SegLimit l;
+    l.q = q >= (uint64_t)kSegLimitNone ? kSegLimitNone - 1u : (uint32_t)q;
+    l.r = (uint32_t)(rel - (q << segbits));
+    return l;
+}
+DPOW_DEV uint32_t seg_limit_at(const SegLimit &l, uint32_t o) { return l.q + (o < l.r ? 1u : 0u); }
+
+template <int NBLK, int W0, int SH>
+DPOW_DEV void seg_invariants(uint32_t (&x)[4][kNC], uint32_t (&p)[kNC], const Launch &L, VarWords<true> &v) {
+#pragma unroll
+    for (int j = 0; j < kNC; ++j) {
+        x[0][j] = L.iv[0]; x[1][j] = L.iv[1]; x[2][j] = L.iv[2]; x[3][j] = L.iv[3];
+    }
+    md5_steps<NBLK, W0, SH, 0, 0, W0 + 1, kNC>(x, L, v);
+    constexpr int I = W0 + 1;
+    constexpr int ai = (64 - I) % 4, bi = (ai + 1) % 4, ci = (ai + 2) % 4, di = (ai + 3) % 4;
+#pragma unroll
+    for (int j = 0; j < kNC; ++j) {
+        p[j] = x[ai][j] + md5_fn<I>(x[bi][j], x[ci][j], x[di][j]);
+        asm volatile("" : "+v"(p[j]), "+v"(x[(64 - W0) % 4][j]));
+        asm volatile("" : "+v"(v.w0km[1][j]), "+v"(v.w0km[2][j]), "+v"(v.w0km[3][j]));
+    }
+}
+
+template <int NBLK, int W0, int SH>
+DPOW_DEV uint64_t hash_wave_block_si(const Launch &L, const KConst &kc, const uint32_t (&xin)[4][kNC],
+                                     const uint32_t (&p)[kNC], const VarWords<true> &v, const uint32_t (&vs)[kNC],
+                                     uint32_t s, uint32_t o, uint32_t lane, uint32_t loff) {
+    constexpr int kLead = VgprK<NBLK, W0, SH, true>::kLead;
+    constexpr int kI0 = W0 + kLead < 62 ? W0 + kLead : 62;
+    static_assert(kLead >= 2, "steps W0 and W0 + 1 precede the hand-ordered pipeline");
+    uint32_t x[4][kNC];
+#pragma unroll
+    for (int j = 0; j < kNC; ++j)
+#pragma unroll
+        for (int w = 0; w < 4; ++w) x[w][j] = xin[w][j];
+    {
+        constexpr int I = W0 + 1;
+        constexpr int ai = (64 - I) % 4, bi = (ai + 1) % 4;
+        const uint32_t km = L.KT[I] + v.seg_d[0];
+#pragma unroll
+        for (int j = 0; j < kNC; ++j) x[ai][j] = x[bi][j] + __builtin_rotateleft32(p[j] + km, md5_shift(I));
+    }
+    md5_steps<NBLK, W0, SH, 0, W0 + 2, kI0, kNC>(x, L, v);
+    pipe::steps<NBLK, W0, SH, 0, kI0, 62>(x, L, v);
+
+    uint64_t bal[kNC];
+    uint64_t any = 0;
+#pragma unroll
+    for (int j = 0; j < kNC; ++j) {
+        bal[j] = __ballot(x[3][j] == L.deq);
+        any |= bal[j];
+    }
+    if (any != 0) {
+        const uint64_t i0 = L.wb_begin + ((uint64_t)s << (24u + L.rbits)) + o;
+#pragma unroll
+        for (int j = 0; j < kNC; ++j) {
+            const uint64_t ij = i0 + 64u * j;
+            uint64_t m = bal[j] & lane_range_mask((int64_t)(L.i_begin - ij), (int64_t)(L.i_end - ij));
+            if (m != 0 && L.ntz > 8u) {
+                const uint32_t sd[3] = {v.seg_d[0], 0u, 0u};
+                const bool ok = ((m >> lane) & 1ull) && full_check<NBLK, W0, SH, true>(L, kc, vs[j], loff, sd);
+                m = __ballot(ok);
+            }
+            if (m != 0) {
+                const uint64_t g = global_of_local(ij + (uint64_t)__builtin_ctzll(m), L.rbits, L.base_tb);
+                if (lane == 0) {
+                    const unsigned long long prev = __hip_atomic_fetch_min(
+                        &L.ctrl->best, (unsigned long long)g, __ATOMIC_RELAXED, __HIP_MEMORY_SCOPE_AGENT);
+                    asm volatile("; dpow: atomicMin performed (%0)" ::"v"(prev));
+                }
+                return g;
+            }
+        }
+    }
+    return kNoHitG;
+}
+
+template <int NBLK, int W0, int SH, bool EQ>
+DPOW_DEV void search_body_si(const Launch &L) {
+    static_assert(NBLK == 1 && SH == 0 && EQ && W0 + 1 != 16 * NBLK - 2,
+                  "segment-inner: one final block, SH = 0, D-equality, W0 + 1 not the bit-length word");
+    if (blockIdx.x == 0) {
+        watcher(L);
+        return;
+    }
+#if DPOW_SI_PAD
+    asm volatile(".rept %0\n s_nop 0\n .endr" ::"i"(DPOW_SI_PAD));
+#endif
+    const uint32_t lane = threadIdx.x & 63u;
+    const uint32_t loff = lane_offset(L.rbits, lane);
+    KConst kc;
+    kconst_init<NBLK, W0, SH, 0, 0, true>(kc, L);
+
+    unsigned long long best = __hip_atomic_load(&L.ctrl->best, __ATOMIC_RELAXED, __HIP_MEMORY_SCOPE_AGENT);
+    best = best < L.bound0 ? best : L.bound0;
+    uint32_t stop = __hip_atomic_load(&L.ctrl->stop, __ATOMIC_RELAXED, __HIP_MEMORY_SCOPE_AGENT);
+
+    __builtin_amdgcn_s_setprio(1);
+    uint32_t x = (blockIdx.x - 1u) % kClaimCounters;
+    const bool skip = stop != 0u || global_of_local(L.i_begin, L.rbits, L.base_tb) >= best;
+    uint64_t claim = skip ? L.n_chunks : claim_next(L.claim + x * kClaimStride, x, lane, 0);
+    const uint32_t segbits = 24u + L.rbits;
+    SegLimit lim = seg_limit_of(L, best);
+    uint32_t pc = L.poll_wb;
+    unsigned long long best_seen = __hip_atomic_load(&L.ctrl->best, __ATOMIC_RELAXED, __HIP_MEMORY_SCOPE_AGENT);
+    uint32_t stop_seen = __hip_atomic_load(&L.ctrl->stop, __ATOMIC_RELAXED, __HIP_MEMORY_SCOPE_AGENT);
+    uint32_t hops = 0;
+    for (;;) {
+        if (claim >= L.n_chunks) {
+            if (skip || ++hops >= kClaimCounters) break;
+            x = (x + 1u) % kClaimCounters;
+            const unsigned long long seen =
+                __hip_atomic_load(L.claim + x * kClaimStride, __ATOMIC_RELAXED, __HIP_MEMORY_SCOPE_AGENT);
+            claim = seen * kClaimCounters + x < L.n_chunks ? claim_next(L.claim + x * kClaimStride, x, lane, 0)
+                                                           : L.n_chunks;
+            continue;
+        }
+        unsigned long long next_v = 0;
+        bool issued = false;
+        const bool big = claim < L.n_big;
+        if (!big) __builtin_amdgcn_s_setprio(0);
+        const uint64_t b_begin = big ? claim * L.chunk : L.n_big * L.chunk + (claim - L.n_big) * L.chunk_tail;
+        const uint32_t csz = big ? L.chunk : L.chunk_tail;
+        const uint32_t nb = (uint32_t)(b_begin + csz < L.n_wblocks ? csz : L.n_wblocks - b_begin);
+        uint32_t o = (uint32_t)(b_begin * (uint64_t)kWaveBlock);
+        bool over = false;
+        for (uint32_t left = nb; left != 0 && stop == 0u; --left, o += (uint32_t)kWaveBlock) {
+            uint32_t s = L.wb_begin + o + (uint64_t)kWaveBlock <= L.i_begin ? 1u : 0u;
+            const uint32_t s_hi =
+                L.n_seg - (L.wb_begin + ((uint64_t)(L.n_seg - 1u) << segbits) + o >= L.i_end ? 1u : 0u);
+            uint32_t s_end = seg_limit_at(lim, o);
+            if (s_end == 0u) {
+                over = true;
+                break;
+            }
+            s_end = s_end < s_hi ? s_end : s_hi;
+            if (left == 1u) {
+                next_v = claim_issue<true>(L.claim + x * kClaimStride, lane);
+                issued = true;
+            }
+            if (s >= s_end) continue;
+            uint32_t vs[kNC];
+            VarWords<true> v;
+            v.kc = &kc;
+            v.seg_d[0] = v.seg_d[1] = v.seg_d[2] = 0u;
+#pragma unroll
+            for (int j = 0; j < kNC; ++j) {
+                vs[j] = wave_uniform_v(L.wb_begin + o + 64u * j, L.rbits, L.base_tb);
+                var_words<SH>(v, j, vs[j], loff, 0u);
+                w0km_fill<W0>(v, j, L);
+            }
+            uint32_t xin[4][kNC], p[kNC];
+            seg_invariants<NBLK, W0, SH>(xin, p, L, v);
+            for (; s < s_end; ++s) {
+                v.seg_d[0] = s;
+#if DPOW_SI_VSEG
+                {
+                    const uint32_t d[3] = {s, 0u, 0u};
+                    kconst_seg<NBLK, W0, SH, 0, 0, true>(kc, L, d);
+                }
+#endif
+                const uint64_t g = hash_wave_block_si<NBLK, W0, SH>(L, kc, xin, p, v, vs, s, o, lane, loff);
+                if (g != kNoHitG) {
+                    best = g < best ? g : best;
+                    lim = seg_limit_of(L, best);
+                    s_end = s;
+                }
+                if (--pc == 0u) {
+                    pc = L.poll_wb;
+                    const bool lower = best_seen < best;
+                    best = lower ? best_seen : best;
+                    stop = stop_seen;
+                    best_seen = __hip_atomic_load(&L.ctrl->best, __ATOMIC_RELAXED, __HIP_MEMORY_SCOPE_AGENT);
+                    stop_seen = __hip_atomic_load(&L.ctrl->stop, __ATOMIC_RELAXED, __HIP_MEMORY_SCOPE_AGENT);
+                    if (lower) {
+                        lim = seg_limit_of(L, best);
+                        const uint32_t e = seg_limit_at(lim, o);
+                        s_end = e < s_end ? e : s_end;
+                    }
+                    if (stop != 0u) s_end = s;
+                }
+            }
+        }
+        if (stop != 0u || over || !issued) break;
+        claim = claim_take(next_v, x, 0);
+    }
+    asm volatile("s_waitcnt vmcnt(0)" ::: "memory");
+    __builtin_amdgcn_fence(__ATOMIC_RELEASE, "workgroup");
+    __syncthreads();
+    if (threadIdx.x == 0) {
+        const uint32_t prev = __hip_atomic_fetch_add(&L.ctrl->done, 1u, __ATOMIC_RELAXED, __HIP_MEMORY_SCOPE_AGENT);
+        if (prev + 1u == L.done_target) publish(L.ctrl, L.snap, L.seq, L.claim, L.ctrl_next);
+    }
+}
+#define DPOW_SEARCH_BODY(NBLK, W0, SH, EQ, KSPAN) search_body_si<NBLK, W0, SH, EQ>(L)
+#else
+#define DPOW_SEARCH_BODY(NBLK, W0, SH, EQ, KSPAN) search_body<NBLK, W0, SH, EQ, KSPAN>(L)
+#endif
+
 template <int NBLK, int W0, int SH, bool EQ, bool KSPAN>
 __global__ void __launch_bounds__(kBlockThreads) __attribute__((amdgpu_num_sgpr(DPOW_NUM_SGPR)))
 md5_search_kernel(const Launch L) {
-    search_body<NBLK, W0, SH, EQ, KSPAN>(L);
+    DPOW_SEARCH_BODY(NBLK, W0, SH, EQ, KSPAN);
 }
 
 template <int NBLK, int W0, int SH, bool EQ, bool KSPAN>
 __global__ void __launch_bounds__(kBlockThreads) __attribute__((amdgpu_num_sgpr(DPOW_NUM_SGPR_LONG)))
 md5_search_kernel_lsgpr(const Launch L) {
-    search_body<NBLK, W0, SH, EQ, KSPAN>(L);
+    DPOW_SEARCH_BODY(NBLK, W0, SH, EQ, KSPAN);
 }
 
 template <int NBLK, int W0, int SH, bool EQ, bool KSPAN>
 __global__ void __launch_bounds__(kBlockThreads) __attribute__((amdgpu_num_sgpr(DPOW_NUM_SGPR_W15)))
 md5_search_kernel_w15sgpr(const Launch L) {
-    search_body<NBLK, W0, SH, EQ, KSPAN>(L);
-}
-
-}
-}
+    DPOW_SEARCH_BODY(NBLK, W0, SH, EQ, KSPAN);
+}
+
+}
+}
diff --git a/distributed-proof-of-work_amd/csrc/md5_variant.hip b/distributed-proof-of-work_amd/csrc/md5_variant.hip
--- a/distributed-proof-of-work_amd/csrc/md5_variant.hip
+++ b/distributed-proof-of-work_amd/csrc/md5_variant.hip
@@ -23,7 +23,15 @@
 }
 #define DPOW_K(w, e, nar) \
     kernel_of<DPOW_VNBLK, w, DPOW_VSH, e, !(DPOW_VSH == 3 && nar && narrow_knobs(DPOW_VNBLK, w).on)>()
-#if DPOW_VNBLK == 1
+#if DPOW_VSI
+#if DPOW_VNBLK != 1 || DPOW_VSH != 0
+#error "the segment-inner unit is built for NBLK = 1, SH = 0"
+#endif
+constexpr int kW0Lo = 0;
+const KernelFn kTable[1][1][4] = {
+    {{DPOW_K(0, true, false), DPOW_K(1, true, false), DPOW_K(2, true, false), DPOW_K(3, true, false)}}};
+#define DPOW_ROW(e, n)
+#elif DPOW_VNBLK == 1
 constexpr int kW0Lo = 0;
 #define DPOW_ROW(e, n)                                                                                              \
     {DPOW_K(0, e, n), DPOW_K(1, e, n), DPOW_K(2, e, n),  DPOW_K(3, e, n),  DPOW_K(4, e, n),  DPOW_K(5, e, n),        \
@@ -42,12 +50,17 @@
 constexpr int kW0N = sizeof(kTable[0][0]) / sizeof(kTable[0][0][0]);
 
 KernelFn pick(int w0, bool eq, bool narrow) {
+#if DPOW_VSI
+    return eq && w0 >= kW0Lo && w0 < kW0Lo + kW0N ? kTable[0][0][w0 - kW0Lo] : nullptr;
+#endif
     return (w0 >= kW0Lo && w0 < kW0Lo + kW0N) ? kTable[eq ? 1 : 0][narrow ? 1 : 0][w0 - kW0Lo] : nullptr;
 }
 }
 
 #if DPOW_VLS
 #define DPOW_SFX _ls
+#elif DPOW_VSI
+#define DPOW_SFX _si
 #else
 #define DPOW_SFX
 #endif
@@ -75,7 +88,7 @@
 }
 
 hipError_t DPOW_NAME(variant_occupancy_, DPOW_VNBLK, DPOW_VSH)(int w0, int *blocks_per_cu) {
-    KernelFn fn = pick(w0, false, true);
+    KernelFn fn = pick(w0, DPOW_VSI != 0, true);
     if (!fn) return hipErrorInvalidValue;
     return hipOccupancyMaxActiveBlocksPerMultiprocessor(blocks_per_cu, reinterpret_cast<const void *>(fn),
                                                         kBlockThreads, 0);
diff --git a/distributed-proof-of-work_amd/csrc/md5_variants.h b/distributed-proof-of-work_amd/csrc/md5_variants.h
--- a/distributed-proof-of-work_amd/csrc/md5_variants.h
+++ b/distributed-proof-of-work_amd/csrc/md5_variants.h
@@ -19,6 +19,7 @@
 DPOW_DECL_VARIANT(2, 3)
 DPOW_DECL_VARIANT(1, 0_ls)
 DPOW_DECL_VARIANT(2, 0_ls)
+DPOW_DECL_VARIANT(1, 0_si)
 #undef DPOW_DECL_VARIANT
 
 inline bool variant_exists(int nblk, int w0, int sh) {
@@ -28,6 +29,9 @@
     return false;
 }
 
+inline bool seg_inner_exists(int nblk, int w0, int sh) {
+    return w0 >= 0 && seg_inner_layout((uint32_t)nblk, (uint32_t)w0, (uint32_t)sh);
+}
 hipError_t search_launch(int nblk, int w0, int sh, const Launch &L, uint32_t grid, hipStream_t stream);
 hipError_t search_occupancy(int nblk, int w0, int sh, int *blocks_per_cu);
 hipError_t search_prepare();
diff --git a/distributed-proof-of-work_amd/csrc/plan.cpp b/distributed-proof-of-work_amd/csrc/plan.cpp
--- a/distributed-proof-of-work_amd/csrc/plan.cpp
+++ b/distributed-proof-of-work_amd/csrc/plan.cpp
@@ -168,8 +168,15 @@
 void candidate_words(const PlannedLaunch &pl, uint64_t local_idx, uint32_t words[32]) {
     const Launch &Lh = pl.L;
     for (uint32_t w = 0; w < 16 * pl.info.nblk; ++w) words[w] = Lh.T[w];
-    const uint64_t i0 = local_idx & ~63ull;
+    uint64_t i0 = local_idx & ~63ull;
     const uint32_t lane = (uint32_t)(local_idx & 63u);
+    uint32_t seg_of_idx = (uint32_t)((local_idx >> Lh.rbits) >> 24);
+    if (Lh.n_seg != 0u) {
+        const uint32_t segbits = 24u + Lh.rbits;
+        const uint64_t rel = i0 - Lh.wb_begin;
+        i0 = Lh.wb_begin + (rel & ((1ull << segbits) - 1ull));
+        seg_of_idx = Lh.seg_first + (uint32_t)(rel >> segbits);
+    }
     const uint32_t V = wave_uniform_v(i0, Lh.rbits, Lh.base_tb) + lane_offset(Lh.rbits, lane);
     const uint32_t sh = pl.info.sh, w0 = pl.info.w0;
     words[w0] += V << (8 * sh);
@@ -188,7 +195,7 @@
     }
     {
         uint32_t d1, d2;
-        const uint32_t seg = (uint32_t)((local_idx >> Lh.rbits) >> 24);
+        const uint32_t seg = seg_of_idx;
         seg_word_deltas(Lh.T[w0 + 1], Lh.T[w0 + 2], seg, Lh.seg_first, sh, d1, d2);
         words[w0 + 1] += d1;
         if (sh == 3 && w0 + 2 != 16 * pl.info.nblk - 2) words[w0 + 2] += d2;
@@ -277,6 +284,64 @@
     return 0;
 }
 
+bool seg_inner_select(WindowPlanner &planner, PlannedLaunch &pl, uint32_t ntz, int mode) {
+    constexpr uint64_t kSeg = 1ull << 24;
+    if (mode == 0 || pl.k0 || pl.L.lspan) return false;
+    if (!seg_inner_layout(pl.info.nblk, pl.info.w0, pl.info.sh) || !use_d_equality(pl.info.nblk, ntz)) return false;
+    if (pl.info.k_begin < kSeg || pl.info.k_end - pl.info.k_begin < 2 * kSeg) return false;
+    if (mode < 0) {
+        const uint64_t expect = expected_first_hit(ntz, pl.L.rbits);
+        if (expect != ~0ull) {
+            const uint64_t max_seg = ((expect / kSegInnerShare) >> pl.L.rbits) / kSeg;
+            if (max_seg < 2) return false;
+            if (pl.info.k_end - pl.info.k_begin > max_seg * kSeg) {
+                planner.restart(pl.info.k_begin, max_seg * kSeg);
+                planner.next(pl);
+            }
+        }
+    }
+    return true;
+}
+
+int seg_inner_size(PlannedLaunch &pl, uint64_t max_blocks, uint64_t *worker_blocks_out) {
+    Launch &L = pl.L;
+    constexpr uint64_t wpb = kBlockThreads / 64;
+    const uint32_t segbits = 24u + L.rbits;
+    const uint64_t seg_lo = pl.info.k_begin >> 24, seg_hi = (pl.info.k_end - 1) >> 24;
+    const uint64_t n_seg = seg_hi - seg_lo + 1;
+    if (n_seg < 2 || n_seg > 0xFFFFFFFFull || L.seg_first != (uint32_t)seg_lo) return DPOW_EINVAL;
+    L.n_seg = (uint32_t)n_seg;
+    L.wb_begin = seg_lo << segbits;
+    L.n_wblocks = (1ull << segbits) / (uint64_t)kWaveBlock;
+    uint64_t chunk = L.chunk / n_seg, chunk_tail = L.chunk_tail / n_seg;
+    while (chunk & (chunk - 1)) chunk &= chunk - 1;
+    while (chunk_tail & (chunk_tail - 1)) chunk_tail &= chunk_tail - 1;
+    if (chunk < 1) chunk = 1;
+    if (chunk_tail < 1) chunk_tail = 1;
+    if (chunk_tail > chunk) chunk_tail = chunk;
+    uint64_t worker_blocks = (L.n_wblocks + wpb - 1) / wpb;
+    if (worker_blocks > max_blocks) worker_blocks = max_blocks;
+    const uint64_t tail_wb = worker_blocks * wpb * kTailClaimsPerWave * chunk_tail;
+    const uint64_t n_big = L.n_wblocks > tail_wb ? (L.n_wblocks - tail_wb) / chunk : 0;
+    const uint64_t rest = L.n_wblocks - n_big * chunk;
+    const uint64_t n_chunks = n_big + (rest + chunk_tail - 1) / chunk_tail;
+    uint64_t need_blocks = (n_chunks + wpb - 1) / wpb;
+    if (need_blocks < n_chunks && need_blocks < kClaimCounters)
+        need_blocks = n_chunks < kClaimCounters ? n_chunks : kClaimCounters;
+    if (worker_blocks > need_blocks) worker_blocks = need_blocks;
+    const uint64_t min_blocks = n_chunks < kClaimCounters ? n_chunks : kClaimCounters;
+    if (worker_blocks < min_blocks && min_blocks <= max_blocks) worker_blocks = min_blocks;
+    if (worker_blocks < kClaimCounters && worker_blocks < n_chunks) return DPOW_EINVAL;
+    L.chunk = (uint32_t)chunk;
+    L.chunk_tail = (uint32_t)chunk_tail;
+    L.n_big = n_big;
+    L.n_chunks = n_chunks;
+    L.n_head = 2 * worker_blocks * wpb;
+    L.n_static = 0;
+    *worker_blocks_out = worker_blocks;
+    return 0;
+}
+
 uint64_t grid_share(uint64_t active, const LaunchKnobs &knobs) {
     const uint64_t cap = knobs.share_max ? knobs.share_max : kShareMax;
     return std::max<uint64_t>(1, std::min(active, cap));
diff --git a/distributed-proof-of-work_amd/csrc/plan.h b/distributed-proof-of-work_amd/csrc/plan.h
--- a/distributed-proof-of-work_amd/csrc/plan.h
+++ b/distributed-proof-of-work_amd/csrc/plan.h
@@ -118,6 +118,7 @@
 
 struct LaunchKnobs {
     uint32_t bpc = 0, min_chunk = 0, cpw = 0, poll_wb = 0;
+    int seg_inner = -1;
     uint32_t share_launch_us = 0;
     uint32_t share_max = 0;
 };
@@ -139,6 +140,10 @@
 constexpr int64_t kShareLaunchNs = (int64_t)DPOW_SHARE_LAUNCH_US * 1000;
 constexpr double kEstRate = 2.3e11;
 uint64_t grid_share(uint64_t active, const LaunchKnobs &knobs);
+
+constexpr uint64_t kSegInnerShare = 64;
+bool seg_inner_select(WindowPlanner &planner, PlannedLaunch &pl, uint32_t ntz, int mode);
+int seg_inner_size(PlannedLaunch &pl, uint64_t max_blocks, uint64_t *worker_blocks);
 bool cap_shared_launch(WindowPlanner &planner, PlannedLaunch &pl, uint64_t active, const LaunchKnobs &knobs);
 
 }
diff --git a/include/dpow_diag.h b/include/dpow_diag.h
--- a/include/dpow_diag.h
+++ b/include/dpow_diag.h
@@ -24,11 +24,19 @@
     uint32_t wave_block;
     uint64_t n_static;
     uint32_t poll_wb;
-    uint32_t pad;
+    uint32_t n_seg;
 } dpow_diag_launch;
 int dpow_diag_launch_geometry(const uint8_t *nonce, size_t nonce_len, uint32_t ntz, uint32_t worker_byte,
                               uint32_t worker_bits, uint64_t k_begin, uint64_t k_end, uint32_t cus,
                               uint32_t share, dpow_diag_launch *out, size_t max_launches);
+
+int dpow_diag_seg_inner_geometry(const uint8_t *nonce, size_t nonce_len, uint32_t ntz, uint32_t worker_byte,
+                                 uint32_t worker_bits, uint64_t k_begin, uint64_t k_end, uint32_t cus, int mode,
+                                 dpow_diag_launch *out, size_t max_launches);
+int dpow_diag_seg_inner_candidate(const uint8_t *nonce, size_t nonce_len, uint32_t ntz, uint32_t worker_byte,
+                                  uint32_t worker_bits, uint64_t k_begin, uint64_t k_end, int mode,
+                                  uint64_t local_idx, uint32_t iv_out[4], uint32_t words_out[32],
+                                  uint32_t *nblk_out);
 
 uint64_t dpow_diag_blocks_per_cu(uint64_t candidates, uint32_t ntz, uint32_t worker_bits);
 
```

New measurement: 229.9 GH/s (median of 6 runs). 1.05x the previous value.
